# researchmm/MM-Diffusion

Hardware: AMD Instinct MI355X
Metric: denoising steps/sec (video+audio pair), 16x64x64 / 25600 (higher is better)
Workload: dtype bf16; 1 GPU; BASELINE configs[1]: Landscape base model (133.68M params), DDPM p_sample, timestep_respacing=250, per-GPU batch 4, 16x3x64x64 video + 1x25600 audio; global_batch=4, parallelism=batch-sharded x1, no in-loop collective, weights=key-seeded synthetic (mm_diffusion.synth), graph_replay=True, batch_lanes=2, finite=True, ranks_seen=1

## Files before the change

include/mmd.h:

```cpp
#ifndef MMD_H
#define MMD_H
#include <stdint.h>
#ifdef __cplusplus
extern "C" {
#endif

#define MMD_F32 0
#define MMD_BF16 1
#define MMD_OK 0
#define MMD_ERR_ARG (-1)
#define MMD_ERR_LAUNCH (-2)
#define MMD_ERR_UNSUPPORTED (-3)

int mmd_version(void);
const char* mmd_last_error(void);
int mmd_debug_install_crash_handler(void);

int mmd_graph_begin(void* stream);
int mmd_graph_end(void* stream, void** exec_out);
int mmd_graph_launch(void* exec, void* stream);
int mmd_graph_destroy(void* exec);
int mmd_stream_create(void** stream_out);
int mmd_stream_sync(void* stream);
int mmd_stream_destroy(void* stream);
int mmd_event_create(void** ev);
int mmd_event_record(void* ev, void* stream);
int mmd_stream_wait_event(void* stream, void* ev);
int mmd_event_elapsed_ms(void* ev_start, void* ev_stop, float* ms);
int mmd_event_destroy(void* ev);

int mmd_temb_fwd(const void* t, int t_kind, int N, int dim, const float* W0, const float* b0, const float* W2,
                 const float* b2, float* out_silu, float* out_raw, void* stream);

int mmd_linear_fwd(const float* x, const float* W, const float* b, float* y, int N, int K, int J, void* stream);

int64_t mmd_gn_workspace_bytes(int dtype, int C, int S, int Tn);
int mmd_gn_stats(int dtype, const void* x, int64_t ld, int C, int S, int Tn, int inner, int64_t outer_stride,
                 int64_t inner_stride, int64_t tstride, const float* gamma, const float* beta, const float* film,
                 int64_t film_ld, float eps, float* a_out, float* b_out, float* mr_out, void* workspace, void* stream);
int mmd_gn_finalize_stats(const float* rec, int64_t rec_ld, int C, int S, int Tn, const float* gamma, const float* beta,
                          const float* film, int64_t film_ld, float eps, float* a_out, float* b_out, float* mr_out, void* stream);
int mmd_gn_apply(int dtype, const void* x, int64_t ldx, void* y, int64_t ldy, int64_t rows, int C, int S, int Tn, int inner,
                 int64_t outer_stride, int64_t inner_stride, int64_t tstride, const float* a, const float* b, int act,
                 void* stream);
int mmd_add_rowbias(int dtype, void* x, int64_t ld, int64_t rows, int C, int64_t rows_per_sample, const float* e,
                    int64_t e_ld, void* stream);
int mmd_colsum_slices(int dtype, const void* dY, int64_t lddy, int S, int64_t Tn, int C, float* out, int64_t ldo, void* stream);

int mmd_conv_gemm(int dtype, const void* A, int64_t lda, const void* W, const float* bias, const void* R, int64_t ldr,
                  void* Y, int64_t ldy, int M, int Cout, int Cin, int ntaps, const int* taps, int D0, int D1, int D2, int tile,
                  void* stream);

int mmd_gn_conv1x1(int dtype, const void* A, int64_t lda, const float* gn_a, const float* gn_b, int act, int S,
                   int64_t rows_per_slice, const void* W, const float* bias, const void* R, int64_t ldr, void* Y, int64_t ldy,
                   int M, int Cout, int Cin, int tile, void* stream);

int mmd_gn_small(int dtype, const void* x, int64_t ldx, void* y, int64_t ldy, int C, int S, int Tn, int inner, int64_t outer_stride,
                 int64_t inner_stride, int64_t tstride, const float* gamma, const float* beta, float eps, int act, void* stream);

int mmd_gn_group(int dtype, const void* x, int64_t ldx, void* y, int64_t ldy, int C, int S, int Tn, int inner, int64_t outer_stride,
                 int64_t inner_stride, int64_t tstride, const float* gamma, const float* beta, const float* film, int64_t film_ld,
                 float eps, int act, float* a_out, float* b_out, float* mr_out, void* stream);

int mmd_zero(void* ptr, int64_t bytes, void* stream);

int mmd_conv_gemm_stats(int dtype, const void* A, int64_t lda, const void* W, const float* bias, const void* R, int64_t ldr,
                        void* Y, int64_t ldy, int M, int Cout, int Cin, int ntaps, const int* taps, int D0, int D1, int D2, int tile,
                        float* stats, int64_t stats_ld, void* stream);
int mmd_gn_conv1x1_stats(int dtype, const void* A, int64_t lda, const float* gn_a, const float* gn_b, int act, int S,
                         int64_t rows_per_slice, const void* W, const float* bias, const void* R, int64_t ldr, void* Y, int64_t ldy,
                         int M, int Cout, int Cin, int tile, float* stats, int64_t stats_ld, void* stream);

int mmd_gn_conv_gemm(int dtype, const void* A, int64_t lda, const float* gn_a, const float* gn_b, int act, int S,
                     int64_t rows_per_slice, const void* W, const float* bias, const void* R, int64_t ldr, void* Y, int64_t ldy,
                     int M, int Cout, int Cin, int ntaps, const int* taps, int D0, int D1, int D2, int tile, void* stream);

int64_t mmd_vconv2d1d_weight_bytes(int Cin);
int mmd_vconv2d1d_pack(const void* Ws, const void* Wt, void* out, int Cin, int Cout, void* stream);
int mmd_vconv2d1d(const void* X, int64_t ldx, const float* gn_a, const float* gn_b, int act, int S, int64_t rows_per_slice,
                  const void* Wf, const float* bias_s, const float* bias_t, void* Y, int64_t ldy, int N, int F, int H, int W,
                  int Cin, int Cout, float* stats, int64_t stats_ld, void* stream);

int64_t mmd_tattn_weight_bytes(int C, int with_pre);
int mmd_tattn_pack(const void* Wpre, const void* Wqkv, const void* Wproj, void* out, int C, void* stream);
int mmd_tattn_block(const void* X, int64_t ldx, const void* A, int64_t lda, void* MID, int64_t ldm, const void* Wf,
                    const float* bias_pre, const float* bias_qkv, const float* bias_proj, const float* gamma, const float* beta,
                    float eps, void* Y, int64_t ldy, int N, int F, int HW, int C, int heads, float* stats, int64_t stats_ld,
                    void* stream);

int64_t mmd_tconv_weight_bytes(int Cin, int Cout);
int mmd_tconv_pack(const void* W, void* out, int Cin, int Cout, void* stream);
int mmd_tconv(const void* X, int64_t ldx, const void* Wf, const float* bias, void* Y, int64_t ldy, int N, int F, int HW, int Cin,
              int Cout, float* stats, int64_t stats_ld, void* stream);

int mmd_aconv(const void* X, int64_t ldx, const void* W, const float* bias, const float* ga, const float* gb, int act, void* Y, int64_t ldy,
              int M, int L, int Cin, int Cout, int dil, float* stats, int64_t stats_ld, void* stream);

int mmd_attn_fwd(int dtype, const void* Q, int64_t ldq, int q_off, const void* KV, int64_t ldkv, int k_off, int v_off, void* O,
                 int64_t ldo, int heads, int ch, int nb, int G, int64_t q_rows_per_batch, int q_per_group,
                 int64_t k_rows_per_batch, int k_per_group, int win, const int* shift_dev, int impl, void* stream);
int mmd_attn_small_fwd(int dtype, const void* QKV, int64_t ld, void* O, int64_t ldo, int C, int heads, int S, int Tn, int inner,
                       int64_t outer_stride, int64_t inner_stride, int64_t tstride, void* stream);

int mmd_resample(int dtype, const void* x, int64_t ldx, void* y, int64_t ldy, int C, int NF, int H, int W, int fh, int fw,
                 int mode, float scale, void* stream);
int mmd_resample_stats(const void* x, int64_t ldx, void* y, int64_t ldy, int C, int NF, int H, int W, int fh, int fw, int mode,
                       float* stats, int64_t stats_ld, void* stream);
int mmd_copy2d(const void* x, int64_t ldx_bytes, void* y, int64_t ldy_bytes, int64_t rows, int64_t row_bytes, void* stream);

int mmd_stem_conv(int dtype, const float* x, const float* w, const float* bias, void* y, int64_t ldy, int N, int F, int Cin,
                  int H, int W, int Cout, int ntaps, const int* taps, void* stream);
int mmd_head_conv(int dtype, const void* x, int64_t ldx, const float* w, const float* bias, float* y, int N, int F, int Cin,
                  int H, int W, int Co, int ntaps, const int* taps, void* stream);
int64_t mmd_head_gemm_weight_bytes(int Cin);
int64_t mmd_head_gemm_workspace_bytes(int64_t M, int ntaps, int Co);
int mmd_head_gemm(const void* x, int64_t ldx, int64_t M, int Cin, const float* gn_a, const float* gn_b, int S, int64_t gn_rows, int act,
                  const void* wimg, float* P, int NO, void* stream);
int mmd_head_gather(const float* P, const float* bias, float* y, int N, int F, int H, int W, int Co, int ntaps, const int* taps,
                    void* stream);

int mmd_ddpm_update(const float* x, const float* model_out, const float* noise, float* out, float* x0_out, float* mean_out,
                    float* logvar_out, const float* tables, const int64_t* t, int T, int N, int F, int C, int HW, int flags,
                    void* stream);
int mmd_q_sample(const float* x0, const float* eps, float* out, const float* tab2, const int64_t* t, int T, int N,
                 int64_t per_sample, void* stream);

int64_t mmd_loss_workspace_bytes(int N);
int mmd_loss_terms(const float* x0, const float* xt, const float* model_out, const float* target, const float* tables,
                   const int64_t* t, int T, int N, int F, int C, int HW, int flags, float vb_scale, float* mse_out, float* vb_out,
                   void* workspace, void* stream);

int mmd_conv_wgrad(int dtype, const void* dY, int64_t lddy, const void* X, int64_t ldx, float* dW, float* db, int M, int Cout, int Cin,
                   int ntaps, const int* taps, int D0, int D1, int D2, int torch_layout, void* stream);
int mmd_pack_blocks(int Cout, int Cin, int nt);
int mmd_pack_conv_weights(int dtype, const void* descs_dev, int n, int total_blocks, void* stream);
int mmd_unpack_conv_grads(const void* descs_dev, int n, int total_blocks, void* stream);
int mmd_gn_bwd(int dtype, const void* x, int64_t ldx, const void* dy, int64_t lddy, void* dx, int64_t lddx, int64_t rows, int C, int S,
               int Tn, int inner, int64_t outer_stride, int64_t inner_stride, int64_t tstride, const float* a, const float* b,
               const float* mr, const float* gamma, const float* beta, const float* film, int64_t film_ld, int act, float* dgamma,
               float* dbeta, float* dfilm, int64_t dfilm_ld, float* workspace, void* stream);
int mmd_gn_bwd_ws0(int dtype, const void* x, int64_t ldx, const void* dy, int64_t lddy, void* dx, int64_t lddx, int64_t rows, int C, int S,
                   int Tn, int inner, int64_t outer_stride, int64_t inner_stride, int64_t tstride, const float* a, const float* b,
                   const float* mr, const float* gamma, const float* beta, const float* film, int64_t film_ld, int act, float* dgamma,
                   float* dbeta, float* dfilm, int64_t dfilm_ld, float* workspace, void* stream);
int mmd_attn_bwd(int dtype, const void* Q, int64_t ldq, int q_off, const void* KV, int64_t ldkv, int k_off, int v_off, const void* O,
                 int64_t ldo, const void* dO, int64_t lddo, void* dQ, int64_t lddq, int dq_off, void* dKV, int64_t lddkv, int dk_off,
                 int dv_off, float* lse_ws, float* dsum_ws, int heads, int ch, int nb, int G, int q_inner, int64_t q_outer,
                 int64_t q_istride, int64_t q_tstride, int q_total, int q_per_group, int k_inner, int64_t k_outer, int64_t k_istride,
                 int64_t k_tstride, int k_mod, int k_per_group, int win, const int* shift_dev, void* stream);
int mmd_attn_fwd_lse(int dtype, const void* Q, int64_t ldq, int q_off, const void* KV, int64_t ldkv, int k_off, int v_off, void* O,
                     int64_t ldo, int heads, int ch, int nb, int G, int64_t q_rows_per_batch, int q_per_group,
                     int64_t k_rows_per_batch, int k_per_group, int win, const int* shift_dev, float* lse2_out, void* stream);
int mmd_attn_bwd_mfma(const void* Q, int64_t ldq, int q_off, const void* KV, int64_t ldkv, int k_off, int v_off, const void* O,
                      int64_t ldo, const void* dO, int64_t lddo, void* dQ, int64_t lddq, int dq_off, void* dKV, int64_t lddkv,
// ... 35 lines not shown
```

mm-diffusion_amd/build.py:

```python
#!/usr/bin/env python3
import os
import subprocess
import sys

HERE = os.path.dirname(os.path.abspath(__file__))
SRC = os.path.join(HERE, "csrc")
OUT = os.path.join(HERE, "lib", "libmmd.so")
SOURCES = ["mmd_core.hip", "mmd_gemm.hip", "mmd_vconv.hip", "mmd_tattn.hip", "mmd_tconv.hip", "mmd_aconv.hip", "mmd_norm.hip", "mmd_attn.hip", "mmd_misc.hip", "mmd_bwd.hip", "mmd_attn_bwd.hip", "mmd_attn_bwd_mfma.hip"]
FLAGS = ["--offload-arch=gfx950", "-O3", "-std=c++17", "-fPIC", "-ffp-contract=fast", "-Wno-unused-result", "-Wno-inline-asm"]
FLAGS += os.environ.get("MMD_EXTRA_CXXFLAGS", "").split()
NO_PACKED_F32 = ["-Xclang", "-target-feature", "-Xclang", "-packed-fp32-ops"]
FLAGS += NO_PACKED_F32


def _stale():
    if not os.path.exists(OUT):
        return True
    t = os.path.getmtime(OUT)
    deps = [os.path.join(SRC, f) for f in os.listdir(SRC)] + [os.path.abspath(__file__)]
    return any(os.path.getmtime(d) > t for d in deps)


def _llvm_bin():
    cands = [os.environ.get("LLVM_BIN")]
    hipcc = os.environ.get("HIPCC", "/opt/rocm/bin/hipcc")
    try:
        out = subprocess.run([hipcc, "--print-prog-name=llvm-objdump"], stdout=subprocess.PIPE, stderr=subprocess.DEVNULL, timeout=60).stdout.decode().strip()
        if out and os.path.isabs(out):
            cands.append(os.path.dirname(out))
    except (OSError, subprocess.SubprocessError):
        pass
    cands += [os.path.join(os.path.dirname(os.path.dirname(os.path.realpath(hipcc))), "lib", "llvm", "bin"), "/opt/rocm/lib/llvm/bin"]
    for d in cands:
        if d and os.path.exists(os.path.join(d, "llvm-objdump")):
            return d
    raise RuntimeError("build check: llvm-objdump not found (looked in %s); set LLVM_BIN to the LLVM bin directory of the ROCm toolchain"
                       % ", ".join(str(d) for d in cands if d))


def _check_no_packed_f32(path):
    import re
    import tempfile
    llvm = _llvm_bin()
    with tempfile.TemporaryDirectory() as td:
        lib = os.path.join(td, "lib.so")
        os.symlink(os.path.abspath(path), lib)
        subprocess.check_call([os.path.join(llvm, "llvm-objdump"), "--offloading", lib], cwd=td, stdout=subprocess.DEVNULL, stderr=subprocess.DEVNULL)
        cos = sorted(f for f in os.listdir(td) if f.endswith("gfx950"))
        if len(cos) < len(SOURCES) - 1:
            raise RuntimeError("build check: expected >= %d gfx950 code objects in %s, found %d" % (len(SOURCES) - 1, path, len(cos)))
        asm = ""
        for f in cos:
            asm += subprocess.run([os.path.join(llvm, "llvm-objdump"), "-d", "--mcpu=gfx950", os.path.join(td, f)],
                                  stdout=subprocess.PIPE, stderr=subprocess.DEVNULL, check=True).stdout.decode(errors="replace")
    n_mfma = len(re.findall(r"\bv_mfma_", asm))
    bad = re.findall(r"\bv_pk_(?:add|mul|fma)_f32\b", asm)
    if n_mfma == 0:
        raise RuntimeError("build check: the disassembly of %s shows no v_mfma instruction - the check looked at the wrong object" % path)
    if bad:
        raise RuntimeError("build check: %d packed-fp32 instruction(s) (%s ...) in %s: the device pass ignored %s" %
                           (len(bad), bad[0], path, " ".join(NO_PACKED_F32)))


def _check_strip_asm(obj):
    import importlib.util
    spec = importlib.util.spec_from_file_location("strip_asm_check", os.path.join(os.path.dirname(HERE), "tools", "strip_asm_check.py"))
    chk = importlib.util.module_from_spec(spec)
    spec.loader.exec_module(chk)
    chk.LLVM = _llvm_bin()
    n, bad = chk.check(chk.disassemble(obj))
    if n == 0 or bad:
        raise RuntimeError("build check: conv1x1_strip_res_kernel: %d kernels checked, %d violations%s" % (n, len(bad), (": " + bad[0]) if bad else ""))


def build(force=False, verbose=True):
    if not force and not _stale():
        return OUT
    os.makedirs(os.path.dirname(OUT), exist_ok=True)
    hipcc = os.environ.get("HIPCC", "/opt/rocm/bin/hipcc")
    objs = []
    procs = []
    for s in SOURCES:
        o = os.path.join(HERE, "lib", s.replace(".hip", ".o"))
        objs.append(o)
        cmd = [hipcc, *FLAGS, "-c", os.path.join(SRC, s), "-o", o]
        procs.append((cmd, subprocess.Popen(cmd, stdout=subprocess.PIPE, stderr=subprocess.STDOUT)))
    for cmd, p in procs:
        out, _ = p.communicate()
        if p.returncode != 0:
            raise RuntimeError("hipcc failed: %s\n%s" % (" ".join(cmd), out.decode()))
        lines = out.decode().splitlines()
        text = "\n".join(ln for ln in lines if "'-packed-fp32-ops' is not a recognized feature" not in ln).strip()
        if verbose and text:
            print(text)
    tmp = OUT + ".tmp"
    cmd = [hipcc, "--offload-arch=gfx950", "-shared", "-fPIC", "-o", tmp, *objs]
    try:
        subprocess.check_call(cmd)
        _check_no_packed_f32(tmp)
        _check_strip_asm(os.path.join(HERE, "lib", "mmd_gemm.o"))
        os.replace(tmp, OUT)
    finally:
        if os.path.exists(tmp):
            os.remove(tmp)
    if verbose:
        print("built", OUT)
    return OUT


if __name__ == "__main__":
    build(force="--force" in sys.argv)
```

mm-diffusion_amd/csrc/mmd_common.h:

```cpp
#pragma once
#include <hip/hip_runtime.h>
#include <stdint.h>
#include <stdio.h>
#include <stdarg.h>
#include "../../include/mmd.h"

#define MMD_F32 0
#define MMD_BF16 1

#define MMD_OK 0
#define MMD_ERR_ARG (-1)
#define MMD_ERR_LAUNCH (-2)
#define MMD_ERR_UNSUPPORTED (-3)

typedef __attribute__((ext_vector_type(8))) __bf16 bf16x8;
typedef __attribute__((ext_vector_type(4))) __bf16 bf16x4;
typedef __attribute__((ext_vector_type(16))) float f32x16;
typedef __attribute__((ext_vector_type(4))) float f32x4;
typedef __attribute__((ext_vector_type(4))) uint32_t u32x4;
typedef __attribute__((ext_vector_type(2))) uint32_t u32x2;

int mmd_set_error(int code, const char* fmt, ...);
int mmd_check_launch(const char* what);

// ... 4 lines not shown

__device__ __forceinline__ float bf16_bits_to_f32(uint32_t bits16) { return __uint_as_float(bits16 << 16); }
__device__ __forceinline__ uint32_t f32_to_bf16_bits(float f) {
  uint32_t u = __float_as_uint(f);
  if ((u & 0x7fffffffu) > 0x7f800000u) return 0x7fc0u;
  u += 0x7fffu + ((u >> 16) & 1u);
  return u >> 16;
}
__device__ __forceinline__ uint32_t pack_bf16x2(float lo, float hi) {
  return f32_to_bf16_bits(lo) | (f32_to_bf16_bits(hi) << 16);
}

template <typename T> struct Elt;
template <> struct Elt<float> {
  static constexpr int EPV = 4;
  static constexpr int DT = MMD_F32;
  __device__ static __forceinline__ void unpack(const u32x4& v, float* f) {
#pragma unroll
    for (int i = 0; i < 4; ++i) f[i] = __uint_as_float(v[i]);
  }
  __device__ static __forceinline__ u32x4 pack(const float* f) {
    u32x4 v;
#pragma unroll
    for (int i = 0; i < 4; ++i) v[i] = __float_as_uint(f[i]);
    return v;
  }
  __device__ static __forceinline__ float ld(const void* p, int64_t i) { return ((const float*)p)[i]; }
  __device__ static __forceinline__ void st(void* p, int64_t i, float v) { ((float*)p)[i] = v; }
};
template <> struct Elt<__bf16> {
  static constexpr int EPV = 8;
  static constexpr int DT = MMD_BF16;
  __device__ static __forceinline__ void unpack(const u32x4& v, float* f) {
#pragma unroll
    for (int i = 0; i < 4; ++i) {
      f[2 * i] = __uint_as_float(v[i] << 16);
      f[2 * i + 1] = __uint_as_float(v[i] & 0xffff0000u);
    }
  }
  __device__ static __forceinline__ u32x4 pack(const float* f) {
    bf16x8 t;
#pragma unroll
    for (int i = 0; i < 8; ++i) t[i] = (__bf16)f[i];
    return __builtin_bit_cast(u32x4, t);
  }
  __device__ static __forceinline__ float ld(const void* p, int64_t i) {
    return bf16_bits_to_f32(((const uint16_t*)p)[i]);
  }
  __device__ static __forceinline__ void st(void* p, int64_t i, float v) {
    ((__bf16*)p)[i] = (__bf16)v;
  }
};

__device__ __forceinline__ float silu_f(float x) { return x * __builtin_amdgcn_rcpf(1.0f + __expf(-x)); }

__device__ __forceinline__ float wave_sum(float v) {
#pragma unroll
  for (int o = 32; o > 0; o >>= 1) v += __shfl_xor(v, o, 64);
  return v;
}
__device__ __forceinline__ double wave_sum_d(double v) {
#pragma unroll
  for (int o = 32; o > 0; o >>= 1) v += __shfl_xor(v, o, 64);
  return v;
}
__device__ __forceinline__ float wave_max(float v) {
#pragma unroll
  for (int o = 32; o > 0; o >>= 1) v = fmaxf(v, __shfl_xor(v, o, 64));
  return v;
}

template <int CTRL, int ROWS>
__device__ __forceinline__ float dpp_add(float v) {
  return v + __builtin_bit_cast(float, __builtin_amdgcn_update_dpp(0, __builtin_bit_cast(int, v), CTRL, ROWS, 0xf, false));
}
__device__ __forceinline__ float halfwave_total(float v) {
  v = dpp_add<0x128, 0xf>(v);
  v = dpp_add<0x124, 0xf>(v);
  v = dpp_add<0x122, 0xf>(v);
  v = dpp_add<0x121, 0xf>(v);
  return dpp_add<0x142, 0xa>(v);
}


static inline int cdiv(int64_t a, int64_t b) { return (int)((a + b - 1) / b); }

#define MMD_MAX_DEVICES 16
static inline int mmd_device_slot() {
  int d = 0;
  (void)hipGetDevice(&d);
  return d & (MMD_MAX_DEVICES - 1);
}
```

mm-diffusion_amd/csrc/mmd_gemm.hip:

```cpp
#include "mmd_common.h"

struct ConvGemmParams {
  const char* A; int64_t lda;
  const char* W;
  const float* bias;
  const char* R; int64_t ldr;
  char* Y; int64_t ldy;
  int M, Cout, Cin, ntaps;
  int D0, D1, D2;
  const float* gn_a; const float* gn_b;
  int gn_act, gn_S;
  int64_t gn_rows;
  float* stats; int64_t stats_ld;
  int taps[27 * 3];
};

template <int BM, int BN>
__device__ __forceinline__ void epilogue_stats(const ConvGemmParams& p, float (&sum)[BM / 64][8], float (&sq)[BM / 64][8], float* sP, int m0,
                                               int n0, int tid) {
  constexpr int CVN = BN / 8, NREC = BM / 64;
  const int lane = tid & 63, wave = tid >> 6, cg = tid % CVN;
#pragma unroll
  for (int r = 0; r < NREC; ++r)
#pragma unroll
// ... 1143 lines not shown
      __builtin_amdgcn_s_barrier();
      asm volatile("" ::: "memory");
      const int wslot = (c * NT + t) % NWS;
      if (t == NT - 1 && !more && p.R) {
#pragma unroll
        for (int ps = 0; ps < NPASS; ++ps)
          rres[ps] = *(const u32x4*)(e_co < p.Cout ? p.R + (row_of(e_rr + ps * RP) * p.ldr + e_co) * ES : (const char*)g_zero_page);
      }
      auto group = [&](int i) {
        const int t2 = (t + 2) % NT, c2 = c + (t + 2) / NT;
        if (i < 2) {
          if (c2 < nchunk) issue_w1((wslot + 2) % NWS, c2, t2, i);
          else dma_dummy();
        } else if (t < HJ) { if (more) issue_h((c + 1) & 1, c + 1, t); else dma_dummy(); }
        else if (t == NT - 1 && c + 2 < nchunk) issue_gn(c + 2);
        else dma_dummy();
      };
      constexpr int TOFF[9] = {-19, -18, -17, -1, 0, 1, 17, 18, 19};
      int toff = TOFF[t];
      asm volatile("" : "+s"(toff));
      const bool tr_on = GN && more && t >= 2 && t < 2 + NSLOT;
      compute(wslot, c & 1, toff, group, [&](int g) { if (tr_on) transform((c + 1) & 1, c + 1, t - 2, g, 1); });
    }
  }
  asm volatile("s_waitcnt vmcnt(0)" ::: "memory");
  __syncthreads();
  if (p.R) {
#pragma unroll
    for (int ps = 0; ps < NPASS; ++ps) LAUNDER4(rres[ps]);
  }

#pragma unroll
  for (int a = 0; a < 2; ++a)
#pragma unroll
    for (int b2 = 0; b2 < 2; ++b2) {
      const int ml = wr * 64 + b2 * 32 + l31;
#pragma unroll
      for (int q = 0; q < 4; ++q) {
        const int col = wc * 64 + a * 32 + 8 * q + 4 * half;
        f32x4 v = {acc[a][b2][4 * q], acc[a][b2][4 * q + 1], acc[a][b2][4 * q + 2], acc[a][b2][4 * q + 3]};
        *(f32x4*)(sC + ml * LDC + col) = v;
      }
    }
  __syncthreads();
  if (e_co < p.Cout) {
#pragma unroll
    for (int ps = 0; ps < NPASS; ++ps) {
      const int ml = e_rr + ps * RP;
      const int64_t m = row_of(ml);
      float v[8];
      const f32x4 c0 = *(const f32x4*)(sC + ml * LDC + e_cg * 8);
      const f32x4 c1 = *(const f32x4*)(sC + ml * LDC + e_cg * 8 + 4);
#pragma unroll
      for (int j = 0; j < 4; ++j) { v[j] = c0[j] + bs[j]; v[4 + j] = c1[j] + bs[4 + j]; }
      if (p.R) {
        float rf[EPV];
        Elt<T>::unpack(rres[ps], rf);
#pragma unroll
        for (int j = 0; j < EPV; ++j) v[j] += rf[j];
      }
      *(u32x4*)(p.Y + (m * p.ldy + e_co) * ES) = Elt<T>::pack(v);
    }
  }
}

#define STRIP_RES_LOAD(J2, off, base)                                                                                        \
  do {                                                                                                                       \
    if ((J2) == 0) asm volatile("global_load_dwordx4 v[248:251], %0, %1" :: "v"(off), "s"(base) : "v248", "v249", "v250", "v251");  \
    else asm volatile("global_load_dwordx4 v[252:255], %0, %1" :: "v"(off), "s"(base) : "v252", "v253", "v254", "v255");       \
  } while (0)
#define STRIP_RES_UNPACK_ASM(A, B, C, D)                                                                                     \
  "s_waitcnt vmcnt(%8)\n\tv_lshlrev_b32 %0, 16, " A "\n\tv_and_b32 %1, 0xffff0000, " A "\n\tv_lshlrev_b32 %2, 16, " B "\n\tv_and_b32 %3, 0xffff0000, " B \
  "\n\tv_lshlrev_b32 %4, 16, " C "\n\tv_and_b32 %5, 0xffff0000, " C "\n\tv_lshlrev_b32 %6, 16, " D "\n\tv_and_b32 %7, 0xffff0000, " D
#define STRIP_RES_WAIT(J2, rf, n)                                                                                            \
  do {                                                                                                                       \
    if ((J2) == 0)                                                                                                           \
      asm volatile(STRIP_RES_UNPACK_ASM("v248", "v249", "v250", "v251")                                                      \
                   : "=v"(rf[0]), "=v"(rf[1]), "=v"(rf[2]), "=v"(rf[3]), "=v"(rf[4]), "=v"(rf[5]), "=v"(rf[6]), "=v"(rf[7]) : "n"(n));  \
    else                                                                                                                     \
      asm volatile(STRIP_RES_UNPACK_ASM("v252", "v253", "v254", "v255")                                                      \
                   : "=v"(rf[0]), "=v"(rf[1]), "=v"(rf[2]), "=v"(rf[3]), "=v"(rf[4]), "=v"(rf[5]), "=v"(rf[6]), "=v"(rf[7]) : "n"(n));  \
  } while (0)
__host__ __device__ constexpr int wait_imm(int vm) { return (vm & 15) | ((vm >> 4) << 14) | 0x0070; }
template <int KS, int RF, int CC, int GNM, int STM, bool HR>
__device__ __forceinline__ void conv1x1_strip_body(const ConvGemmParams& p, const int nsplit) {
  constexpr int K = 64 * KS;
  constexpr int NCG = 4 * KS;
  constexpr int BR = 128 * RF;
  constexpr int NA = CC / 32;
  constexpr int GP = CC / 32;
  constexpr int PLANE_B = CC * 128, STAGE_B = KS * PLANE_B;
  constexpr bool PIPE = KS >= 4 && !(KS == 4 && HR);
  constexpr bool DEFER = KS > 2 || RF == 1;
  static_assert(RF == 2 || CC == 32, "one row fragment per wave: one sub-tile per chunk, deferred epilogue");
  extern __shared__ __attribute__((aligned(16))) char smem[];
  char* sW = smem;

  const int tid = threadIdx.x;
  const int lane = tid & 63;
  const int wave = __builtin_amdgcn_readfirstlane(tid >> 6);
  const int half = lane >> 5, l31 = lane & 31;

  const int nwg = gridDim.x;
  int wgid;
  {
    const int bid = blockIdx.x, q = nwg >> 3, r = nwg & 7, xcd = bid & 7;
    wgid = (xcd < r ? xcd * (q + 1) : r * (q + 1) + (xcd - r) * q) + (bid >> 3);
  }
  const int sp = wgid % nsplit, mt = wgid / nsplit;
  const int Cs = p.Cout / nsplit, cbase = sp * Cs, nchunk = Cs / CC;
  const int m0 = mt * BR;
  float* sBias = (float*)(smem + 2 * STAGE_B);
  float* sGN = sBias + ((Cs + 3) & ~3);
  float* sRec = sGN + (GNM != 0 ? 4 * K : 0);

  typedef const __attribute__((address_space(1))) void* gptr_t;
  typedef __attribute__((address_space(3))) void* lptr_t;
  const int lrow = lane >> 3, pc = lane & 7;
  const char* w_ptr[GP];
#pragma unroll
  for (int ih = 0; ih < GP; ++ih) {
    const int row = 8 * (ih * 4 + wave) + lrow;
    const int logical = pc ^ ((row >> 1) & 7);
    w_ptr[ih] = p.W + ((int64_t)(cbase + row) * K + logical * 8) * 2;
  }
  const unsigned lds0 = (unsigned)(uintptr_t)(lptr_t)sW;
  auto issue = [&](int stage, int ci) {
    const int64_t off = (int64_t)ci * CC * K * 2;
#pragma unroll
    for (int pl = 0; pl < KS; ++pl)
#pragma unroll
      for (int ih = 0; ih < GP; ++ih)
        asm volatile("s_mov_b32 m0, %1\n\ts_nop 0\n\tglobal_load_lds_dwordx4 %0, off"
                     :: "v"(w_ptr[ih] + off + pl * 128), "s"(lds0 + stage * STAGE_B + pl * PLANE_B + (ih * 4 + wave) * 1024) : "memory", "m0");
  };

  issue(0, 0);
  int rowc[RF];
  bool rok[RF];
  uint32_t yoff[RF], roff[RF];
  u32x4 xa[RF][NCG];
#pragma unroll
  for (int f = 0; f < RF; ++f) {
    const int row = m0 + wave * (32 * RF) + f * 32 + l31;
    rok[f] = row < p.M;
    rowc[f] = rok[f] ? row : p.M - 1;
    yoff[f] = (uint32_t)rowc[f] * (uint32_t)(p.ldy * 2) + 16 * half;
    roff[f] = (uint32_t)rowc[f] * (uint32_t)(p.ldr * 2) + 16 * half;
    if (p.ntaps == 1) {
      const char* ap = p.A + ((int64_t)rowc[f] * p.lda + half * 8) * 2;
#pragma unroll
      for (int cg = 0; cg < NCG; ++cg) xa[f][cg] = *(const u32x4*)(ap + cg * 32);
    } else {
      const int D12 = p.D1 * p.D2;
      const int q2 = rowc[f] % p.D2, q1 = (rowc[f] / p.D2) % p.D1, q0 = (rowc[f] / D12) % p.D0;
#pragma unroll
      for (int pl = 0; pl < KS; ++pl) {
        const int tap = (64 * pl) / p.Cin, ci0 = 64 * pl - tap * p.Cin;
        const int o0 = p.taps[3 * tap], o1 = p.taps[3 * tap + 1], o2 = p.taps[3 * tap + 2];
        const bool ok = (unsigned)(q0 + o0) < (unsigned)p.D0 && (unsigned)(q1 + o1) < (unsigned)p.D1 && (unsigned)(q2 + o2) < (unsigned)p.D2;
        const int64_t src = (int64_t)rowc[f] + (int64_t)o0 * D12 + o1 * p.D2 + o2;
        const char* ap = ok ? p.A + (src * p.lda + ci0 + half * 8) * 2 : (const char*)g_zero_row + half * 16;
#pragma unroll
        for (int c = 0; c < 4; ++c) xa[f][4 * pl + c] = *(const u32x4*)(ap + c * 32);
      }
    }
  }
  constexpr bool gn = GNM != 0;
// ... 96 lines not shown
    auto epi_step = [&](int s_, f32x16 (&ac)[RF], float (&kp)[2][2], int t, bool dma_between, bool last) __attribute__((always_inline)) {
      const int j2 = t / PJ, r = t % PJ;
      const int cb = s_ * 32;
      const int a = s_ % NA, par = (s_ / NA) & 1;
      if (r == 0) {
        if (j2 == 0) {
          eb[1][0] = *(const f32x4*)(sBias + cb + 16 + 8 * half);
          eb[1][1] = *(const f32x4*)(sBias + cb + 16 + 8 * half + 4);
        }
#pragma unroll
        for (int k = 0; k < 4; ++k) eu[k] = 0.f;
      }
      if (r < RF * SPU) {
        const int f = r / SPU, k = r % SPU;
        if (k < 4) {
          if (HR && k == 0) {
            if (last) STRIP_RES_WAIT(j2, erf, 2 * (NU - 1 - (j2 * RF + f)) + (j2 * RF + f));
            else if (dma_between) STRIP_RES_WAIT(j2, erf, 2 * (NU - 1) + D);
            else STRIP_RES_WAIT(j2, erf, 2 * (NU - 1));
          }
          const auto sw = __builtin_amdgcn_permlane32_swap(__float_as_uint(ac[f][8 * j2 + k]), __float_as_uint(ac[f][8 * j2 + 4 + k]), false, false);
          ev[k] = __uint_as_float(sw[0]) + eb[j2][0][k];
          ev[4 + k] = __uint_as_float(sw[1]) + eb[j2][1][k];
          if constexpr (HR) {
            ev[k] += erf[k];
            ev[4 + k] += erf[4 + k];
          }
        } else if (k == 4) {
          epk = Elt<__bf16>::pack(ev);
          *(u32x4*)(p.Y + (int64_t)(cbase + cb + 16 * j2) * 2 + yoff[f]) = epk;
          if (HR && !last) STRIP_RES_LOAD(j2, roff[f], p.R + (int64_t)(cbase + cb + 32 + 16 * j2) * 2);
        } else {
          const int q = k - 5;
          const float r0 = __uint_as_float(epk[q] << 16), r1 = __uint_as_float(epk[q] & 0xffff0000u);
          eu[q >> 1] += r0;
          eu[q >> 1] += r1;
          eu[2 + (q >> 1)] += r0 * r0;
          eu[2 + (q >> 1)] += r1 * r1;
        }
      } else {
        const int h = r - RF * SPU;
        if (h < 4) et[h] = halfwave_total(eu[h]);
        else {
          kp[j2][0] = (l31 & 1) ? et[1] : et[0];
          kp[j2][1] = (l31 & 1) ? et[3] : et[2];
          if (RF == 1) {
            float* d = sRec + ((l31 >> 1) == 8 ? (((par * 4 + wave) * (NA * 2) + a * 2 + j2) * 2 + half) * 4 + (l31 & 1) * 2 : 128 + lane * 2);
            d[0] = kp[j2][0];
            d[1] = kp[j2][1];
          }
        }
      }
    };
    auto block = [&](int s_, f32x16 (&an)[RF], f32x16 (&ap)[RF], float (&kp)[2][2], bool dma_between) __attribute__((always_inline)) {
#pragma unroll
      for (int ks = 0; ks < PF; ++ks) frag_read(s_, ks);
      epi_begin(s_ - 1);
      __builtin_amdgcn_sched_barrier(0);
#pragma unroll
      for (int i = 0; i < NM; ++i) {
        if (i % RF == 0 && i / RF + PF < NKS) frag_read(s_, i / RF + PF);
        mfma_one(i, an);
        __builtin_amdgcn_sched_barrier(0);
#pragma unroll
        for (int t = NSTEP * i / NM; t < NSTEP * (i + 1) / NM; ++t) epi_step(s_ - 1, ap, kp, t, dma_between, false);
        __builtin_amdgcn_sched_barrier(0);
      }
    };
    auto mfma_sub = [&](int s_, f32x16 (&ac)[RF]) __attribute__((always_inline)) {
#pragma unroll
      for (int ks = 0; ks < PF; ++ks) frag_read(s_, ks);
#pragma unroll
      for (int i = 0; i < NM; ++i) {
        if (i % RF == 0 && i / RF + PF < NKS) frag_read(s_, i / RF + PF);
        mfma_one(i, ac);
      }
    };
    auto epi = [&](int s_, f32x16 (&ac)[RF], float (&kp)[2][2], bool dma_between, bool last) __attribute__((always_inline)) {
      epi_begin(s_);
#pragma unroll
      for (int t = 0; t < NSTEP; ++t) epi_step(s_, ac, kp, t, dma_between, last);
    };
    auto commit = [&](int s_, float (&kp)[2][2]) __attribute__((always_inline)) {
      if (STM == 1 && wave_ok && (RF == 2 || (wave & 1) == 0) && (l31 >> 1) == 8) {
        const int a = s_ % NA, par = (s_ / NA) & 1;
#pragma unroll
        for (int j2 = 0; j2 < 2; ++j2) {
          const int col = cbase + s_ * 32 + 16 * j2 + 8 * half;
          float* d = p.stats + (rec * p.stats_ld + (col >> 2) + (l31 & 1)) * 2;
          float o0 = 0.f, o1 = 0.f;
          if (RF == 1) {
            const float* o = sRec + ((((par * 4 + wave + 1) * (NA * 2) + a * 2 + j2) * 2 + half) * 4 + (l31 & 1) * 2);
            o0 = o[0];
            o1 = o[1];
          }
          d[0] = kp[j2][0] + o0;
          d[1] = kp[j2][1] + o1;
        }
      }
    };
    auto boundary = [&](int c) __attribute__((always_inline)) {
      if (c == 1) __builtin_amdgcn_s_waitcnt(wait_imm((NA - 1) * NU * VM_U));
      else __builtin_amdgcn_s_waitcnt(wait_imm(NA * NU * VM_U));
      __builtin_amdgcn_s_barrier();
      asm volatile("" ::: "memory");
      issue((c + 1) & 1, c + 1 < nchunk ? c + 1 : nchunk - 1);
    };
    issue(1, nchunk > 1 ? 1 : 0);
    mfma_sub(0, acc[0]);
    for (int s1 = 1; s1 < NS; s1 += 2) {
      if (NA == 1) {
        boundary(s1);
        if (RF == 1 && s1 >= 2) commit(s1 - 2, keep[1]);
      }
      block(s1, acc[1], acc[0], keep[0], NA == 1);
      if (RF == 2) commit(s1 - 1, keep[0]);
      if (s1 + 1 < NS) {
        boundary((s1 + 1) / NA);
        if (RF == 1) commit(s1 - 1, keep[0]);
        block(s1 + 1, acc[0], acc[1], keep[1], true);
        if (RF == 2) commit(s1, keep[1]);
      }
    }
    auto tail = [&](f32x16 (&ac)[RF], float (&kp)[2][2], float (&kq)[2][2]) __attribute__((always_inline)) {
      epi(NS - 1, ac, kp, false, true);
      if (RF == 2) commit(NS - 1, kp);
      if (RF == 1 && STM == 1) {
        __builtin_amdgcn_s_waitcnt(wait_imm(63));
        __builtin_amdgcn_s_barrier();
        if (NS >= 2) commit(NS - 2, kq);
        commit(NS - 1, kp);
      }
    };
    if ((NS - 1) & 1) tail(acc[1], keep[1], keep[0]);
    else tail(acc[0], keep[0], keep[1]);
    asm volatile("s_waitcnt vmcnt(0)" ::: "memory");
  } else {
  for (int ci = 0; ci < nchunk; ++ci) {
    const int st = ci & 1;
    if (ci + 1 < nchunk) issue(st ^ 1, ci + 1);
    u32x4 outv[RF][2];
    float srec[2][2];
#pragma unroll
    for (int a = 0; a < NA; ++a) {
      const int cb = ci * CC + a * 32;
      u32x4 rres[RF][2];
      if constexpr (HR) {
#pragma unroll
        for (int f = 0; f < RF; ++f)
#pragma unroll
          for (int j2 = 0; j2 < 2; ++j2)
            rres[f][j2] = *(const u32x4*)(p.R + (int64_t)(cbase + cb + 16 * j2) * 2 + roff[f]);
        __builtin_amdgcn_sched_barrier(0);
      }
      f32x16 acc[RF];
#pragma unroll
      for (int f = 0; f < RF; ++f)
#pragma unroll
        for (int r = 0; r < 16; ++r) acc[f][r] = 0.f;
      const char* bW = sW + st * STAGE_B + (a * 32 + l31) * 128;
#pragma unroll
      for (int pl = 0; pl < KS; ++pl)
#pragma unroll
        for (int c = 0; c < 4; ++c) {
          const u32x4 fw = *(const u32x4*)(bW + pl * PLANE_B + (((2 * c + half) ^ xsw) * 16));
#pragma unroll
          for (int f = 0; f < RF; ++f) Mma<__bf16>::run(fw, xa[f][4 * pl + c], acc[f]);
        }
#pragma unroll
      for (int j2 = 0; j2 < 2; ++j2) {
        const int col = cbase + cb + 16 * j2 + 8 * half;
        const f32x4 b0 = *(const f32x4*)(sBias + cb + 16 * j2 + 8 * half), b1 = *(const f32x4*)(sBias + cb + 16 * j2 + 8 * half + 4);
        float u[16];
#pragma unroll
        for (int i = 0; i < 16; ++i) u[i] = 0.f;
#pragma unroll
        for (int f = 0; f < RF; ++f) {
          float v[8];
#pragma unroll
          for (int j = 0; j < 4; ++j) {
            const auto sw = __builtin_amdgcn_permlane32_swap(__float_as_uint(acc[f][8 * j2 + j]), __float_as_uint(acc[f][8 * j2 + 4 + j]),
                                                             false, false);
            v[j] = __uint_as_float(sw[0]);
            v[4 + j] = __uint_as_float(sw[1]);
          }
#pragma unroll
          for (int j = 0; j < 4; ++j) { v[j] += b0[j]; v[4 + j] += b1[j]; }
          if constexpr (HR) {
            float rf[8];
            Elt<__bf16>::unpack(rres[f][j2], rf);
#pragma unroll
            for (int j = 0; j < 8; ++j) v[j] += rf[j];
          }
          const u32x4 pk = Elt<__bf16>::pack(v);
          if (DEFER && a == NA - 1) outv[f][j2] = pk;
          else *(u32x4*)(p.Y + (int64_t)(cbase + cb + 16 * j2) * 2 + yoff[f]) = pk;
          if (STM != 0) {
            float rf[8];
            Elt<__bf16>::unpack(pk, rf);
#pragma unroll
            for (int j = 0; j < 4; ++j) {
              u[0] += rf[j];
              u[1] += rf[4 + j];
              u[2] += rf[j] * rf[j];
              u[3] += rf[4 + j] * rf[4 + j];
            }
          }
        }
        if (STM == 1) {
          const float t0 = halfwave_total(u[0]), t1 = halfwave_total(u[1]), t2 = halfwave_total(u[2]), t3 = halfwave_total(u[3]);
          const float msum = (l31 & 1) ? t1 : t0, msq = (l31 & 1) ? t3 : t2;
          if (RF == 1) {
            if ((l31 >> 1) == 8) {
              float* d = sRec + ((((ci & 1) * 4 + wave) * (NA * 2) + a * 2 + j2) * 2 + half) * 4 + (l31 & 1) * 2;
              d[0] = msum;
              d[1] = msq;
            }
            srec[j2][0] = msum;
            srec[j2][1] = msq;
          } else if (wave_ok && (l31 >> 1) == 8) {
            float* d = p.stats + (rec * p.stats_ld + (col >> 2) + (l31 & 1)) * 2;
            d[0] = msum;
            d[1] = msq;
          }
        }
      }
    }
    __builtin_amdgcn_s_waitcnt(0x0070);
    __builtin_amdgcn_s_barrier();
#pragma unroll
    for (int j2 = 0; DEFER && j2 < 2; ++j2) {
      const int col = cbase + ci * CC + (NA - 1) * 32 + 16 * j2 + 8 * half;
#pragma unroll
      for (int f = 0; f < RF; ++f)
        *(u32x4*)(p.Y + (int64_t)(cbase + ci * CC + (NA - 1) * 32 + 16 * j2) * 2 + yoff[f]) = outv[f][j2];
      if (RF == 1) {
        if (STM == 1 && wave_ok && (wave & 1) == 0 && (l31 >> 1) == 8) {
          const float* o = sRec + ((((ci & 1) * 4 + wave + 1) * (NA * 2) + (NA - 1) * 2 + j2) * 2 + half) * 4 + (l31 & 1) * 2;
          float* d = p.stats + (rec * p.stats_ld + (col >> 2) + (l31 & 1)) * 2;
          d[0] = srec[j2][0] + o[0];
          d[1] = srec[j2][1] + o[1];
        }
      }
    }
  }
  }
}

#define STRIP_LAUNCH_BOUNDS __launch_bounds__(256, (KS <= 2 ? (RF == 1 ? 4 : 3) : 2))
template <int KS, int RF, int CC, int GNM, int STM>
__global__ STRIP_LAUNCH_BOUNDS void conv1x1_strip_kernel(const ConvGemmParams p, const int nsplit) {
  conv1x1_strip_body<KS, RF, CC, GNM, STM, false>(p, nsplit);
}
template <int KS, int RF, int CC, int GNM, int STM>
__global__ STRIP_LAUNCH_BOUNDS __attribute__((amdgpu_num_vgpr(248))) void conv1x1_strip_res_kernel(const ConvGemmParams p, const int nsplit) {
  conv1x1_strip_body<KS, RF, CC, GNM, STM, true>(p, nsplit);
}

template <int KS, int RF, int CC, int GNM, int STM, bool HR>
static int launch_conv1x1_strip_res(const ConvGemmParams& p, hipStream_t st) {
  constexpr int BR = 128 * RF, STAGE_B = KS * CC * 128;
  const int rowblocks = cdiv(p.M, BR), nch = p.Cout / CC;
  static const int want_blocks = [] {
    const char* e = getenv("MMD_STRIP_BLOCKS");
    const int v = e ? atoi(e) : 0;
    return v > 0 ? v : 256;
  }();
  int nsplit = 1;
  for (int d = 1; d <= nch && d <= 16; ++d)
    if (nch % d == 0) {
      nsplit = d;
      if ((int64_t)rowblocks * d >= want_blocks) break;
    }
  const int Cs = p.Cout / nsplit;
  constexpr size_t REC_B = RF == 1 ? 2 * 4 * (CC / 32) * 2 * 32 * sizeof(float) : 0;
  const size_t lds = 2 * (size_t)STAGE_B + (size_t)((Cs + 3) & ~3) * 4 + (p.gn_a ? 4 * (size_t)(64 * KS) * 4 : 0) + REC_B;
  const size_t lds_max = 2 * (size_t)STAGE_B + 2048 * 4 + 4 * (size_t)(64 * KS) * 4 + REC_B;
  if (lds > lds_max) return mmd_set_error(MMD_ERR_UNSUPPORTED, "conv_gemm tile 131 (strip): %d output channels per block", Cs);
  static bool attr_done[MMD_MAX_DEVICES] = {};
  bool& attr_set = attr_done[mmd_device_slot()];
  if (!attr_set) {
    const void* kfn = HR ? (const void*)conv1x1_strip_res_kernel<KS, RF, CC, GNM, STM> : (const void*)conv1x1_strip_kernel<KS, RF, CC, GNM, STM>;
    hipError_t e = hipFuncSetAttribute(kfn, hipFuncAttributeMaxDynamicSharedMemorySize, (int)lds_max);
    if (e != hipSuccess) return mmd_set_error(MMD_ERR_LAUNCH, "conv1x1_strip: set LDS attr: %s", hipGetErrorString(e));
    attr_set = true;
  }
  if (HR) hipLaunchKernelGGL((conv1x1_strip_res_kernel<KS, RF, CC, GNM, STM>), dim3(rowblocks * nsplit), dim3(256), lds, st, p, nsplit);
  else hipLaunchKernelGGL((conv1x1_strip_kernel<KS, RF, CC, GNM, STM>), dim3(rowblocks * nsplit), dim3(256), lds, st, p, nsplit);
  return mmd_check_launch("conv1x1_strip");
}

template <int KS, int RF, int CC, int GNM, int STM>
static int launch_conv1x1_strip_mode(const ConvGemmParams& p, hipStream_t st) {
  return p.R ? launch_conv1x1_strip_res<KS, RF, CC, GNM, STM, true>(p, st) : launch_conv1x1_strip_res<KS, RF, CC, GNM, STM, false>(p, st);
}

template <int KS, int RF, int CC, int STM>
static int launch_conv1x1_strip_st(const ConvGemmParams& p, hipStream_t st) {
  if (!p.gn_a) return launch_conv1x1_strip_mode<KS, RF, CC, 0, STM>(p, st);
  return p.gn_act ? launch_conv1x1_strip_mode<KS, RF, CC, 2, STM>(p, st) : launch_conv1x1_strip_mode<KS, RF, CC, 1, STM>(p, st);
}

template <int KS, int RF, int CC>
static int launch_conv1x1_strip(const ConvGemmParams& p, hipStream_t st) {
  return p.stats ? launch_conv1x1_strip_st<KS, RF, CC, 1>(p, st) : launch_conv1x1_strip_st<KS, RF, CC, 0>(p, st);
}

static int dispatch_conv1x1_strip(const ConvGemmParams& p, hipStream_t st) {
  const int K = p.Cin * p.ntaps;
  const int rf = K <= 256 ? 2 : 1, cc = K <= 256 ? 64 : 32;
  if ((K != 128 && K != 256 && K != 384 && K != 512) || p.Cin % 64 != 0 || p.Cout % cc != 0 ||
      (int64_t)p.M * p.ldy * 2 >= 0xffffffffLL || (p.R && (int64_t)p.M * p.ldr * 2 >= 0xffffffffLL) || (p.gn_a && (p.ntaps != 1 || p.gn_rows < 128 * rf)) ||
      (p.ntaps == 1 && (p.taps[0] || p.taps[1] || p.taps[2])))
    return mmd_set_error(MMD_ERR_UNSUPPORTED, "conv_gemm tile 131 (strip): needs ntaps * Cin in {128, 256, 384, 512}, Cin %% 64 == 0, Cout %% %d == 0, "
                         "fused GroupNorm only for 1x1 convs with slices of >= %d rows (got Cin=%d ntaps=%d Cout=%d)", cc, 128 * rf, p.Cin, p.ntaps, p.Cout);
  if (K == 128) {
    static const bool rf1 = [] { const char* e = getenv("MMD_STRIP_K128_RF1"); return !(e && e[0] == '0'); }();
    if (rf1 && p.gn_a && p.gn_rows >= 16384 && p.ntaps == 1 && p.Cout % 32 == 0) return launch_conv1x1_strip<2, 1, 32>(p, st);
    return launch_conv1x1_strip<2, 2, 64>(p, st);
  }
  if (K == 256) return launch_conv1x1_strip<4, 2, 64>(p, st);
  if (K == 384) return launch_conv1x1_strip<6, 1, 32>(p, st);
  return launch_conv1x1_strip<8, 1, 32>(p, st);
}

template <typename T, bool GN>
static int launch_conv_gemm_halo(const ConvGemmParams& p, hipStream_t st) {
  bool taps_ok = p.ntaps <= 9;
  for (int t = 0; t < p.ntaps && taps_ok; ++t)
    taps_ok = p.taps[t * 3] == 0 && p.taps[t * 3 + 1] >= -1 && p.taps[t * 3 + 1] <= 1 && p.taps[t * 3 + 2] >= -1 && p.taps[t * 3 + 2] <= 1;
  if (!taps_ok || p.D1 % 8 != 0 || p.D2 % 16 != 0 || (int64_t)p.D0 * p.D1 * p.D2 != p.M || p.Cin % (8 * Elt<T>::EPV) != 0)
    return mmd_set_error(MMD_ERR_UNSUPPORTED, "conv_gemm tile 130 (halo): needs spatial taps (|dh|,|dw| <= 1), D1 %% 8 == 0, D2 %% 16 == 0, "
                         "full frames and Cin a multiple of one 128-byte K step");
  if (GN && (p.ntaps != 9 || p.gn_rows % ((int64_t)p.D1 * p.D2) != 0))
    return mmd_set_error(MMD_ERR_UNSUPPORTED, "conv_gemm tile 130 with fused GroupNorm: needs the nine spatial taps and slices of whole frames");
  const size_t lds = 2 * (size_t)(23 * 8 * 128) + 2 * (size_t)(128 * 128) + 336 + (GN ? 1024 : 0);
  static bool attr_done[MMD_MAX_DEVICES] = {};
  bool& attr_set = attr_done[mmd_device_slot()];
  if (!attr_set) {
    hipError_t e = hipFuncSetAttribute((const void*)conv_gemm_halo_kernel<T, GN>, hipFuncAttributeMaxDynamicSharedMemorySize, (int)lds);
    if (e != hipSuccess) return mmd_set_error(MMD_ERR_LAUNCH, "conv_gemm_halo: set LDS attr: %s", hipGetErrorString(e));
    attr_set = true;
  }
  const int grid = (p.M / 128) * cdiv(p.Cout, 128);
  hipLaunchKernelGGL((conv_gemm_halo_kernel<T, GN>), dim3(grid), dim3(256), lds, st, p);
  return mmd_check_launch("conv_gemm_halo");
}

template <bool GN>
static int launch_conv_gemm_halo16(const ConvGemmParams& p, hipStream_t st) {
  bool taps_ok = p.ntaps == 9;
  for (int t = 0; t < p.ntaps && taps_ok; ++t)
    taps_ok = p.taps[t * 3] == 0 && p.taps[t * 3 + 1] == t / 3 - 1 && p.taps[t * 3 + 2] == t % 3 - 1;
  if (!taps_ok || p.D1 % 16 != 0 || p.D2 % 16 != 0 || (int64_t)p.D0 * p.D1 * p.D2 != p.M || p.Cin % 64 != 0 ||
      ((int64_t)p.D1 * p.D2 - 1) * p.lda * 2 + (int64_t)p.Cin * 2 >= 0x7fffffffLL || (int64_t)128 * p.Cin * 9 * 2 >= 0x7fffffffLL)
    return mmd_set_error(MMD_ERR_UNSUPPORTED, "conv_gemm tile 133 (halo, 16 x 16 patches): needs the nine spatial taps in row-major (dh, dw) order, "
                         "D1 %% 16 == 0, D2 %% 16 == 0, full frames, Cin %% 64 == 0 and frames below 2 GB");
  if (GN && p.gn_rows % ((int64_t)p.D1 * p.D2) != 0)
    return mmd_set_error(MMD_ERR_UNSUPPORTED, "conv_gemm tile 133 with fused GroupNorm: needs slices of whole frames");
  constexpr size_t OPS_B = 2 * (size_t)(41 * 8 * 128) + 3 * (size_t)(128 * 128), C_B = 256 * 132 * sizeof(float);
  const size_t lds = (OPS_B > C_B ? OPS_B : C_B) + 1024 + 256;
  static bool attr_done[MMD_MAX_DEVICES] = {};
  bool& attr_set = attr_done[mmd_device_slot()];
  if (!attr_set) {
    hipError_t e = hipFuncSetAttribute((const void*)conv_gemm_halo16_kernel<GN>, hipFuncAttributeMaxDynamicSharedMemorySize, (int)lds);
    if (e != hipSuccess) return mmd_set_error(MMD_ERR_LAUNCH, "conv_gemm_halo16: set LDS attr: %s", hipGetErrorString(e));
    attr_set = true;
  }
  const int grid = (p.M / 256) * cdiv(p.Cout, 128);
  hipLaunchKernelGGL((conv_gemm_halo16_kernel<GN>), dim3(grid), dim3(512), lds, st, p);
  return mmd_check_launch("conv_gemm_halo16");
}

template <typename T>
static bool glds_desc_ok(const ConvGemmParams& p) {
  static const bool on = [] { const char* e = getenv("MMD_GEMM_DESC"); return !(e && e[0] == '0'); }();
  constexpr int ES = 16 / Elt<T>::EPV;
  int maxshift = 0;
  for (int t = 0; t < p.ntaps; ++t) {
    const int64_t sh = ((int64_t)p.taps[3 * t] * p.D1 * p.D2 + (int64_t)p.taps[3 * t + 1] * p.D2 + p.taps[3 * t + 2]) * p.lda * ES;
    if (sh > 0x3fffffff || sh < -0x3fffffff) return false;
    (void)maxshift;
  }
  return on && ((int64_t)p.M * p.lda + p.Cin) * ES < 0x7fffffffLL && (int64_t)128 * p.Cin * p.ntaps * ES < 0x7fffffffLL;
}

template <typename T>
static int launch_conv_gemm_glds(const ConvGemmParams& p, hipStream_t st) {
  const size_t lds = 128 * 132 * sizeof(float) + 336;
  static bool attr_done[MMD_MAX_DEVICES] = {};
  bool& attr_set = attr_done[mmd_device_slot()];
  if (!attr_set) {
    hipError_t e = hipFuncSetAttribute((const void*)conv_gemm_glds_kernel<T, false, 2, false>, hipFuncAttributeMaxDynamicSharedMemorySize, (int)lds);
    if (e == hipSuccess) e = hipFuncSetAttribute((const void*)conv_gemm_glds_kernel<T, true, 2, false>, hipFuncAttributeMaxDynamicSharedMemorySize, (int)lds);
    if (e == hipSuccess) e = hipFuncSetAttribute((const void*)conv_gemm_glds_kernel<T, true, 2, true>, hipFuncAttributeMaxDynamicSharedMemorySize, (int)lds);
    if (e != hipSuccess) return mmd_set_error(MMD_ERR_LAUNCH, "conv_gemm_glds: set LDS attr: %s", hipGetErrorString(e));
    attr_set = true;
  }
  const int grid = cdiv(p.M, 128) * cdiv(p.Cout, 128);
  if (p.Cin % (8 * Elt<T>::EPV) != 0) hipLaunchKernelGGL((conv_gemm_glds_kernel<T, false, 2, false>), dim3(grid), dim3(256), lds, st, p);
  else if (glds_desc_ok<T>(p)) hipLaunchKernelGGL((conv_gemm_glds_kernel<T, true, 2, true>), dim3(grid), dim3(256), lds, st, p);
  else hipLaunchKernelGGL((conv_gemm_glds_kernel<T, true, 2, false>), dim3(grid), dim3(256), lds, st, p);
  return mmd_check_launch("conv_gemm_glds");
}

template <typename T>
static int launch_conv_gemm_ring(const ConvGemmParams& p, hipStream_t st) {
  if (p.Cin % (8 * Elt<T>::EPV) != 0)
    return mmd_set_error(MMD_ERR_UNSUPPORTED, "conv_gemm tile 132 (deep ring): Cin must be a multiple of one 128-byte K step");
  const size_t lds = 8 * (size_t)(128 * 128) + 336;
  static bool attr_done[MMD_MAX_DEVICES] = {};
  bool& attr_set = attr_done[mmd_device_slot()];
  if (!attr_set) {
    hipError_t e = hipFuncSetAttribute((const void*)conv_gemm_glds_kernel<T, true, 4, false>, hipFuncAttributeMaxDynamicSharedMemorySize, (int)lds);
    if (e == hipSuccess) e = hipFuncSetAttribute((const void*)conv_gemm_glds_kernel<T, true, 4, true>, hipFuncAttributeMaxDynamicSharedMemorySize, (int)lds);
    if (e != hipSuccess) return mmd_set_error(MMD_ERR_LAUNCH, "conv_gemm_ring: set LDS attr: %s", hipGetErrorString(e));
    attr_set = true;
  }
  const int grid = cdiv(p.M, 128) * cdiv(p.Cout, 128);
  if (glds_desc_ok<T>(p)) hipLaunchKernelGGL((conv_gemm_glds_kernel<T, true, 4, true>), dim3(grid), dim3(256), lds, st, p);
  else hipLaunchKernelGGL((conv_gemm_glds_kernel<T, true, 4, false>), dim3(grid), dim3(256), lds, st, p);
  return mmd_check_launch("conv_gemm_ring");
}

template <typename T, int BM, int BN, bool GN>
static int launch_conv_gemm(const ConvGemmParams& p, hipStream_t st) {
  const size_t lds_ops = 2 * (size_t)(BM + BN) * ROWB;
  const size_t lds_c = (size_t)BM * (BN + 4) * sizeof(float);
  const size_t lds = (lds_ops > lds_c ? lds_ops : lds_c) + 336 + (GN ? 16 * 256 : 0);
  static bool attr_done[MMD_MAX_DEVICES] = {};
  bool& attr_set = attr_done[mmd_device_slot()];
  if (!attr_set) {
    hipError_t e = hipFuncSetAttribute((const void*)conv_gemm_kernel<T, BM, BN, GN>,
                                       hipFuncAttributeMaxDynamicSharedMemorySize, (int)lds);
    if (e != hipSuccess) return mmd_set_error(MMD_ERR_LAUNCH, "conv_gemm: set LDS attr: %s", hipGetErrorString(e));
    attr_set = true;
  }
  const int grid = cdiv(p.M, BM) * cdiv(p.Cout, BN);
  hipLaunchKernelGGL((conv_gemm_kernel<T, BM, BN, GN>), dim3(grid), dim3(256), lds, st, p);
  return mmd_check_launch("conv_gemm");
}

template <typename T>
static int dispatch_conv_gemm(const ConvGemmParams& p, int tile, hipStream_t st) {
  if (tile == 133) {
    if constexpr (Elt<T>::EPV == 8) return p.gn_a ? launch_conv_gemm_halo16<true>(p, st) : launch_conv_gemm_halo16<false>(p, st);
    else return mmd_set_error(MMD_ERR_UNSUPPORTED, "conv_gemm tile 133: bf16 only");
  }
  if (p.gn_a) {
    if (tile == 130) {
      if constexpr (Elt<T>::EPV == 8) return launch_conv_gemm_halo<T, true>(p, st);
      else return mmd_set_error(MMD_ERR_UNSUPPORTED, "conv_gemm tile 130 with fused GroupNorm: bf16 only");
    }
    if (tile == 128) return launch_conv_gemm<T, 128, 128, true>(p, st);
    return launch_conv_gemm<T, 64, 64, true>(p, st);
  }
  if (tile == 129) return launch_conv_gemm_glds<T>(p, st);
  if (tile == 132) return launch_conv_gemm_ring<T>(p, st);
  if (tile == 130) return launch_conv_gemm_halo<T, false>(p, st);
  if (tile == 128) return launch_conv_gemm<T, 128, 128, false>(p, st);
  return launch_conv_gemm<T, 64, 64, false>(p, st);
}

static int conv_gemm_impl(int dtype, const void* A, int64_t lda, const void* W, const float* bias, const void* R, int64_t ldr,
                          void* Y, int64_t ldy, int M, int Cout, int Cin, int ntaps, const int* taps, int D0, int D1, int D2,
                          int tile, const float* gn_a, const float* gn_b, int gn_act, int gn_S, int64_t gn_rows, float* stats,
                          int64_t stats_ld, void* stream) {
  const int epv = dtype == MMD_BF16 ? 8 : 4;
  MMD_REQUIRE(dtype == MMD_BF16 || dtype == MMD_F32, "conv_gemm: bad dtype %d", dtype);
  MMD_REQUIRE(A && W && Y && M > 0 && Cout > 0 && Cin > 0, "conv_gemm: null/empty argument");
  MMD_REQUIRE(ntaps >= 1 && ntaps <= 27 && taps, "conv_gemm: ntaps %d out of [1,27]", ntaps);
  MMD_REQUIRE(Cin % epv == 0, "conv_gemm: Cin %d must be a multiple of %d", Cin, epv);
  MMD_REQUIRE(Cout % 8 == 0, "conv_gemm: Cout %d must be a multiple of 8", Cout);
  MMD_REQUIRE(lda % epv == 0 && ldy % epv == 0 && (!R || ldr % epv == 0), "conv_gemm: row strides must be 16-byte multiples");
  MMD_REQUIRE(((uintptr_t)A | (uintptr_t)W | (uintptr_t)Y | (uintptr_t)R) % 16 == 0, "conv_gemm: pointers must be 16-byte aligned");
  MMD_REQUIRE(D0 > 0 && D1 > 0 && D2 > 0, "conv_gemm: bad position dims");
  MMD_REQUIRE(!gn_a || (gn_b && (ntaps == 1 || tile == 130 || tile == 133) && gn_S > 0 && gn_rows >= 128 && (Cin <= 256 || tile == 131 || tile == 130 || tile == 133) &&
                        (int64_t)gn_S * gn_rows == M),
              "gn_conv1x1 / gn_conv_gemm: needs contiguous slices of >= 128 rows covering M, Cin <= 256 unless tile 130 / 131, taps only with tile 130 "
              "(got S=%d rows=%ld Cin=%d M=%d ntaps=%d tile=%d)", gn_S, (long)gn_rows, Cin, M, ntaps, tile);
  ConvGemmParams p;
  p.A = (const char*)A; p.lda = lda; p.W = (const char*)W; p.bias = bias;
  p.R = (const char*)R; p.ldr = ldr; p.Y = (char*)Y; p.ldy = ldy;
  p.M = M; p.Cout = Cout; p.Cin = Cin; p.ntaps = ntaps; p.D0 = D0; p.D1 = D1; p.D2 = D2;
  p.gn_a = gn_a; p.gn_b = gn_b; p.gn_act = gn_act; p.gn_S = gn_S; p.gn_rows = gn_rows;
  MMD_REQUIRE(!stats || (M % 64 == 0 && Cout % 4 == 0 && stats_ld >= Cout / 4 && tile != 130 && tile != 133 && (uintptr_t)stats % 8 == 0),
              "conv_gemm: output statistics need M %% 64 == 0, Cout %% 4 == 0, stats_ld >= Cout / 4 (quads) and a row-tiled main loop (not tiles 130 / 133)");
  p.stats = stats; p.stats_ld = stats_ld;
  for (int i = 0; i < ntaps * 3; ++i) p.taps[i] = taps[i];
  hipStream_t st = (hipStream_t)stream;
  if (tile == 0) tile = (int64_t)cdiv(M, 128) * cdiv(Cout, 128) >= 320 ? 128 : 64;
  MMD_REQUIRE(tile == 64 || tile == 128 || ((tile == 129 || tile == 132) && !gn_a) || (tile == 130 && (!gn_a || dtype == MMD_BF16)) ||
                  ((tile == 131 || tile == 133) && dtype == MMD_BF16),
              "conv_gemm: tile must be 0, 64, 128, 129 (128 direct-to-LDS), 130 (halo-tile 3x3), 131 (row strip, bf16 1x1 convs) or 132 (129 with a "
              "four-slot ring for launches of few tiles)");
  if (tile == 131) return dispatch_conv1x1_strip(p, st);
  return dtype == MMD_BF16 ? dispatch_conv_gemm<__bf16>(p, tile, st) : dispatch_conv_gemm<float>(p, tile, st);
}

extern "C" int mmd_conv_gemm(int dtype, const void* A, int64_t lda, const void* W, const float* bias, const void* R, int64_t ldr,
                             void* Y, int64_t ldy, int M, int Cout, int Cin, int ntaps, const int* taps, int D0, int D1, int D2,
                             int tile, void* stream) {
  return conv_gemm_impl(dtype, A, lda, W, bias, R, ldr, Y, ldy, M, Cout, Cin, ntaps, taps, D0, D1, D2, tile, nullptr, nullptr, 0, 0,
                        0, nullptr, 0, stream);
}

extern "C" int mmd_conv_gemm_stats(int dtype, const void* A, int64_t lda, const void* W, const float* bias, const void* R, int64_t ldr,
                                   void* Y, int64_t ldy, int M, int Cout, int Cin, int ntaps, const int* taps, int D0, int D1, int D2,
                                   int tile, float* stats, int64_t stats_ld, void* stream) {
  MMD_REQUIRE(stats, "conv_gemm_stats: null statistics buffer");
  return conv_gemm_impl(dtype, A, lda, W, bias, R, ldr, Y, ldy, M, Cout, Cin, ntaps, taps, D0, D1, D2, tile, nullptr, nullptr, 0, 0,
                        0, stats, stats_ld, stream);
}

extern "C" int mmd_gn_conv1x1(int dtype, const void* A, int64_t lda, const float* gn_a, const float* gn_b, int act, int S,
                              int64_t rows_per_slice, const void* W, const float* bias, const void* R, int64_t ldr, void* Y,
                              int64_t ldy, int M, int Cout, int Cin, int tile, void* stream) {
  static const int tap0[3] = {0, 0, 0};
  MMD_REQUIRE(gn_a && gn_b, "gn_conv1x1: null GroupNorm affine");
  return conv_gemm_impl(dtype, A, lda, W, bias, R, ldr, Y, ldy, M, Cout, Cin, 1, tap0, 1, 1, 1, tile, gn_a, gn_b, act, S,
                        rows_per_slice, nullptr, 0, stream);
}

extern "C" int mmd_gn_conv1x1_stats(int dtype, const void* A, int64_t lda, const float* gn_a, const float* gn_b, int act, int S,
                                    int64_t rows_per_slice, const void* W, const float* bias, const void* R, int64_t ldr, void* Y,
                                    int64_t ldy, int M, int Cout, int Cin, int tile, float* stats, int64_t stats_ld, void* stream) {
  static const int tap0[3] = {0, 0, 0};
  MMD_REQUIRE(gn_a && gn_b && stats, "gn_conv1x1_stats: null GroupNorm affine / statistics buffer");
  return conv_gemm_impl(dtype, A, lda, W, bias, R, ldr, Y, ldy, M, Cout, Cin, 1, tap0, 1, 1, 1, tile, gn_a, gn_b, act, S,
                        rows_per_slice, stats, stats_ld, stream);
}

extern "C" int mmd_gn_conv_gemm(int dtype, const void* A, int64_t lda, const float* gn_a, const float* gn_b, int act, int S,
                                int64_t rows_per_slice, const void* W, const float* bias, const void* R, int64_t ldr, void* Y,
                                int64_t ldy, int M, int Cout, int Cin, int ntaps, const int* taps, int D0, int D1, int D2, int tile,
                                void* stream) {
  MMD_REQUIRE(gn_a && gn_b, "gn_conv_gemm: null GroupNorm affine");
  MMD_REQUIRE(tile == 130 || tile == 133, "gn_conv_gemm: the fused input GroupNorm of a conv with taps exists on the halo tiles (130 / 133) only");
  return conv_gemm_impl(dtype, A, lda, W, bias, R, ldr, Y, ldy, M, Cout, Cin, ntaps, taps, D0, D1, D2, tile, gn_a, gn_b, act, S,
                        rows_per_slice, nullptr, 0, stream);
}
```

mm-diffusion_amd/csrc/mmd_norm.hip:

```cpp
#include "mmd_common.h"

#define GN_GROUPS 32
typedef __attribute__((ext_vector_type(2))) double f64x2;

struct SliceGeom {
  int S, Tn, inner;
  int64_t outer_stride, inner_stride, tstride;
};

__device__ __forceinline__ int64_t slice_base(const SliceGeom& g, int s) {
  return (int64_t)(s / g.inner) * g.outer_stride + (int64_t)(s % g.inner) * g.inner_stride;
}
__device__ __forceinline__ int slice_of_row(const SliceGeom& g, int64_t m) {
  const int64_t o = m / g.outer_stride, rem = m % g.outer_stride;
  return (int)(o * g.inner + (rem / g.inner_stride) % g.inner);
}

template <typename T, bool ONE>
__global__ __launch_bounds__(256) void gn_partial_kernel(const char* __restrict__ x, int64_t ld, int C, SliceGeom g, int R,
                                                         double* __restrict__ part, int nchunks,
                                                         const float* __restrict__ gamma, const float* __restrict__ beta,
                                                         const float* __restrict__ film, int64_t film_ld, float eps,
                                                         float* __restrict__ a_out, float* __restrict__ b_out, float* __restrict__ mr_out) {
  constexpr int EPV = Elt<T>::EPV;
  constexpr int ES = 16 / EPV;
  __shared__ float s_sum[2048];
  __shared__ float s_sq[2048];
  __shared__ float s_mean[GN_GROUPS], s_rstd[GN_GROUPS];
  const int s = blockIdx.y, chunk = blockIdx.x, tid = threadIdx.x;
  const int CV = C / EPV;
  const int CVB = min(CV, 256);
  const int RPP = 256 / CVB;
  const int col0 = tid % CVB, rl = tid / CVB;
  const int j0 = chunk * R;
  const int j1 = min(j0 + R, g.Tn);
  const int64_t base = slice_base(g, s);
  const int cpg = C / GN_GROUPS;
  for (int cp = 0; cp < CV; cp += 256) {
  const int col = col0 + cp;
  if (col >= CV) break;
  float sum[EPV], sq[EPV];
#pragma unroll
  for (int j = 0; j < EPV; ++j) sum[j] = sq[j] = 0.f;
  float piv[EPV];
  {
    const int c0 = col * EPV;
    const int g0 = c0 / cpg;
    int gc = g0, rem = c0 - g0 * cpg;
#pragma unroll
    for (int e = 0; e < EPV; ++e) {
      piv[e] = Elt<T>::ld(x, base * ld + (int64_t)gc * cpg);
      if (++rem == cpg) { rem = 0; ++gc; }
    }
  }
  if (rl < RPP) {
    const char* xp = x + (base * ld + (int64_t)col * EPV) * ES;
    const int64_t rstride = g.tstride * ld * ES;
    for (int jb = j0 + rl; jb < j1; jb += 4 * RPP) {
      u32x4 v[4];
#pragma unroll
      for (int u = 0; u < 4; ++u) {
        const int j = jb + u * RPP;
        if (j < j1) v[u] = *(const u32x4*)(xp + (int64_t)j * rstride);
      }
#pragma unroll
      for (int u = 0; u < 4; ++u) {
        if (jb + u * RPP < j1) {
          float f[EPV];
          Elt<T>::unpack(v[u], f);
#pragma unroll
          for (int e = 0; e < EPV; ++e) { const float d = f[e] - piv[e]; sum[e] += d; sq[e] += d * d; }
        }
      }
    }
#pragma unroll
    for (int e = 0; e < EPV; ++e) {
      s_sum[rl * C + col * EPV + e] = sum[e];
      s_sq[rl * C + col * EPV + e] = sq[e];
    }
  }
  }
  __syncthreads();
  {
    const int gi = tid >> 3, k = tid & 7;
    const int n = RPP * cpg;
// ... 294 lines not shown
  int R = 4 * rpp;
  while (cdiv(Tn, R) > cap / 4 && R < 1024) R *= 2;
  return R;
}

extern "C" int64_t mmd_gn_workspace_bytes(int dtype, int C, int S, int Tn) {
  if (C <= 0 || S <= 0 || Tn <= 0) return 0;
  return (int64_t)S * cdiv(Tn, gn_rows_per_block(dtype, C, S, Tn)) * GN_GROUPS * 2 * sizeof(double);
}

extern "C" int mmd_gn_stats(int dtype, const void* x, int64_t ld, int C, int S, int Tn, int inner, int64_t outer_stride,
                            int64_t inner_stride, int64_t tstride, const float* gamma, const float* beta,
                            const float* film, int64_t film_ld, float eps, float* a_out, float* b_out, float* mr_out,
                            void* workspace, void* stream) {
  int rc = check_geom("gn_stats", dtype, C, S, Tn, inner);
  if (rc) return rc;
  MMD_REQUIRE(x && gamma && beta && a_out && b_out, "gn_stats: null pointer");
  MMD_REQUIRE(((uintptr_t)x) % 16 == 0 && ld % (dtype == MMD_BF16 ? 8 : 4) == 0, "gn_stats: x must be 16-byte aligned rows");
  SliceGeom g{S, Tn, inner, outer_stride, inner_stride, tstride};
  hipStream_t st = (hipStream_t)stream;
  const int R = gn_rows_per_block(dtype, C, S, Tn);
  const int nchunks = cdiv(Tn, R);
  if (nchunks == 1) {
    if (dtype == MMD_BF16)
      hipLaunchKernelGGL((gn_partial_kernel<__bf16, true>), dim3(1, S), dim3(256), 0, st, (const char*)x, ld, C, g, R, (double*)nullptr, 1,
                         gamma, beta, film, film_ld, eps, a_out, b_out, mr_out);
    else
      hipLaunchKernelGGL((gn_partial_kernel<float, true>), dim3(1, S), dim3(256), 0, st, (const char*)x, ld, C, g, R, (double*)nullptr, 1,
                         gamma, beta, film, film_ld, eps, a_out, b_out, mr_out);
    return mmd_check_launch("gn_stats_one");
  }
  MMD_REQUIRE(workspace && ((uintptr_t)workspace) % 16 == 0, "gn_stats: 16-byte aligned workspace required for multi-block slices");
  dim3 grid(nchunks, S);
  if (dtype == MMD_BF16)
    hipLaunchKernelGGL((gn_partial_kernel<__bf16, false>), grid, dim3(256), 0, st, (const char*)x, ld, C, g, R, (double*)workspace, nchunks,
                       gamma, beta, film, film_ld, eps, a_out, b_out, (float*)nullptr);
  else
    hipLaunchKernelGGL((gn_partial_kernel<float, false>), grid, dim3(256), 0, st, (const char*)x, ld, C, g, R, (double*)workspace, nchunks,
                       gamma, beta, film, film_ld, eps, a_out, b_out, (float*)nullptr);
  rc = mmd_check_launch("gn_partial");
  if (rc) return rc;
  hipLaunchKernelGGL(gn_finalize_kernel, dim3(S), dim3(1024), 0, st, (const char*)x, dtype, ld, g, (const double*)workspace, nchunks, C, Tn, gamma, beta,
                     film, film_ld, eps, a_out, b_out, mr_out);
  return mmd_check_launch("gn_finalize");
}

__global__ __launch_bounds__(256) void gn_finalize_rec_kernel(const float* __restrict__ rec, int64_t rec_ld, int C, int S, int Tn,
                                                              const float* __restrict__ gamma, const float* __restrict__ beta,
                                                              const float* __restrict__ film, int64_t film_ld, float eps,
                                                              float* __restrict__ a_out, float* __restrict__ b_out, float* __restrict__ mr_out) {
  __shared__ double s_a[4], s_b[4];
  const int gi = blockIdx.x, s = blockIdx.y, tid = threadIdx.x;
  const int cpg = C / GN_GROUPS, qpg = cpg / 4;
  const int nrec = Tn / 64;
  const float* base = rec + ((int64_t)s * nrec * rec_ld + (int64_t)gi * qpg) * 2;
  const int total = nrec * qpg;
  const int c = gi * cpg + min(tid, cpg - 1);
  const float gv = gamma[c], bv0 = beta[c];
  float fsc = 0.f, fsh = 0.f;
  if (film) {
    fsc = film[(int64_t)s * film_ld + c];
    fsh = film[(int64_t)s * film_ld + C + c];
  }
  double a[4] = {0.0, 0.0, 0.0, 0.0}, b[4] = {0.0, 0.0, 0.0, 0.0};
  for (int i = tid; i < total; i += 1024) {
#pragma unroll
    for (int u = 0; u < 4; ++u) {
      const int k = i + 256 * u;
      const int kk = min(k, total - 1);
      const int r = kk / qpg, cq = kk - r * qpg;
      const float2 v = *(const float2*)(base + ((int64_t)r * rec_ld + cq) * 2);
      const double m = k < total ? 1.0 : 0.0;
      a[u] += m * (double)v.x;
      b[u] += m * (double)v.y;
    }
  }
  double ta = (a[0] + a[1]) + (a[2] + a[3]), tb = (b[0] + b[1]) + (b[2] + b[3]);
  ta = wave_sum_d(ta);
  tb = wave_sum_d(tb);
  if ((tid & 63) == 0) { s_a[tid >> 6] = ta; s_b[tid >> 6] = tb; }
  __syncthreads();
  if (tid < cpg) {
    const double sa = (s_a[0] + s_a[1]) + (s_a[2] + s_a[3]), sb = (s_b[0] + s_b[1]) + (s_b[2] + s_b[3]);
    const double cnt = (double)Tn * (double)cpg;
    const double mean = sa / cnt;
    double var = sb / cnt - mean * mean;
    if (var < 0.0) var = 0.0;
    const float mean_f = (float)mean, rstd_f = (float)(1.0 / sqrt(var + (double)eps));
    if (mr_out && tid == 0) {
      mr_out[((int64_t)s * GN_GROUPS + gi) * 2] = mean_f;
      mr_out[((int64_t)s * GN_GROUPS + gi) * 2 + 1] = rstd_f;
    }
    float av = rstd_f * gv;
    float bv = bv0 - mean_f * av;
    if (film) {
      const float sc = 1.f + fsc;
      av *= sc;
      bv = bv * sc + fsh;
    }
    a_out[(int64_t)s * C + c] = av;
    b_out[(int64_t)s * C + c] = bv;
  }
}

extern "C" int mmd_gn_finalize_stats(const float* rec, int64_t rec_ld, int C, int S, int Tn, const float* gamma, const float* beta,
                                     const float* film, int64_t film_ld, float eps, float* a_out, float* b_out, float* mr_out,
                                     void* stream) {
  MMD_REQUIRE(rec && gamma && beta && a_out && b_out, "gn_finalize_stats: null pointer");
  MMD_REQUIRE(C > 0 && C % (4 * GN_GROUPS) == 0 && C / GN_GROUPS <= 256 && rec_ld >= C / 4,
              "gn_finalize_stats: channel count %d (groups of whole quads: a multiple of 128; ld %ld quads)", C, (long)rec_ld);
  MMD_REQUIRE(S > 0 && Tn > 0 && Tn % 64 == 0, "gn_finalize_stats: slices must be multiples of 64 rows (S=%d Tn=%d)", S, Tn);
  hipLaunchKernelGGL(gn_finalize_rec_kernel, dim3(GN_GROUPS, S), dim3(256), 0, (hipStream_t)stream, rec, rec_ld, C, S, Tn, gamma, beta,
                     film, film_ld, eps, a_out, b_out, mr_out);
  return mmd_check_launch("gn_finalize_stats");
}

template <typename T>
__global__ __launch_bounds__(256) void gn_group_kernel(const char* __restrict__ x, int64_t ldx, char* __restrict__ y, int64_t ldy, int C,
                                                       SliceGeom g, const float* __restrict__ gamma, const float* __restrict__ beta,
                                                       const float* __restrict__ film, int64_t film_ld, float eps, int act,
                                                       float* __restrict__ a_out, float* __restrict__ b_out, float* __restrict__ mr_out) {
  constexpr int ES = sizeof(T), MAXI = 16;
  __shared__ float s_red[2][4];
  __shared__ float s_ab[2][64];
  const int gi = blockIdx.x, s = blockIdx.y, tid = threadIdx.x;
  const int cpg = C / GN_GROUPS, qpg = cpg / 4, items = g.Tn * qpg;
  const int64_t base = slice_base(g, s);
  const char* xg = x + (int64_t)gi * cpg * ES;
  float f[MAXI][4];
#pragma unroll
  for (int j = 0; j < MAXI; ++j) {
    const int i = tid + 256 * j;
    if (i < items) {
      const int r = i / qpg, k = i - r * qpg;
      const char* q = xg + ((base + (int64_t)r * g.tstride) * ldx + 4 * k) * ES;
      if constexpr (ES == 2) {
        const u32x2 v = *(const u32x2*)q;
        f[j][0] = __uint_as_float(v[0] << 16); f[j][1] = __uint_as_float(v[0] & 0xffff0000u);
        f[j][2] = __uint_as_float(v[1] << 16); f[j][3] = __uint_as_float(v[1] & 0xffff0000u);
      } else {
        const f32x4 v = *(const f32x4*)q;
        f[j][0] = v[0]; f[j][1] = v[1]; f[j][2] = v[2]; f[j][3] = v[3];
      }
    } else {
      f[j][0] = f[j][1] = f[j][2] = f[j][3] = 0.f;
    }
  }
  auto block_sum = [&](float v, int slot) {
    v = wave_sum(v);
    if ((tid & 63) == 0) s_red[slot][tid >> 6] = v;
    __syncthreads();
    return (s_red[slot][0] + s_red[slot][1]) + (s_red[slot][2] + s_red[slot][3]);
  };
  float t = 0.f;
#pragma unroll
  for (int j = 0; j < MAXI; ++j) t += (f[j][0] + f[j][1]) + (f[j][2] + f[j][3]);
  const float inv_cnt = 1.f / ((float)g.Tn * (float)cpg);
  const float mean = block_sum(t, 0) * inv_cnt;
  t = 0.f;
#pragma unroll
  for (int j = 0; j < MAXI; ++j)
    if (tid + 256 * j < items) {
      const float d0 = f[j][0] - mean, d1 = f[j][1] - mean, d2 = f[j][2] - mean, d3 = f[j][3] - mean;
      t += (d0 * d0 + d1 * d1) + (d2 * d2 + d3 * d3);
    }
  const float var = block_sum(t, 1) * inv_cnt;
  const float rstd = (float)(1.0 / sqrt((double)var + (double)eps));
  if (tid < cpg) {
    const int c = gi * cpg + tid;
    float av = rstd * gamma[c];
    float bv = beta[c] - mean * av;
    if (film) {
      const float sc = 1.f + film[(int64_t)s * film_ld + c];
      av *= sc;
      bv = bv * sc + film[(int64_t)s * film_ld + C + c];
    }
    if (a_out) {
      a_out[(int64_t)s * C + c] = av;
      b_out[(int64_t)s * C + c] = bv;
    }
    s_ab[0][tid] = av;
// ... 110 lines not shown
```

mm-diffusion_amd/mm_diffusion/_hip.py:

```python
import ctypes as C
import gc
import os

import torch

_HERE = os.path.dirname(os.path.abspath(__file__))
LIB_PATH = os.environ.get("MMD_LIB") or os.path.join(os.path.dirname(_HERE), "lib", "libmmd.so")

F32, BF16 = 0, 1
_lib = None

i32, i64, f32, vp = C.c_int, C.c_int64, C.c_float, C.c_void_p


_PROTOS = {
    "mmd_version": (C.c_int, []),
    "mmd_last_error": (C.c_char_p, []),
    "mmd_debug_install_crash_handler": (i32, []),
    "mmd_graph_begin": (i32, [vp]),
    "mmd_graph_end": (i32, [vp, C.POINTER(vp)]),
    "mmd_graph_launch": (i32, [vp, vp]),
    "mmd_graph_destroy": (i32, [vp]),
    "mmd_stream_create": (i32, [C.POINTER(vp)]),
    "mmd_stream_sync": (i32, [vp]),
    "mmd_stream_destroy": (i32, [vp]),
    "mmd_event_create": (i32, [C.POINTER(vp)]),
    "mmd_event_record": (i32, [vp, vp]),
    "mmd_stream_wait_event": (i32, [vp, vp]),
    "mmd_event_elapsed_ms": (i32, [vp, vp, C.POINTER(f32)]),
    "mmd_event_destroy": (i32, [vp]),
    "mmd_temb_fwd": (i32, [vp, i32, i32, i32, vp, vp, vp, vp, vp, vp, vp]),
    "mmd_linear_fwd": (i32, [vp, vp, vp, vp, i32, i32, i32, vp]),
    "mmd_gn_workspace_bytes": (i64, [i32, i32, i32, i32]),
    "mmd_gn_stats": (i32, [i32, vp, i64, i32, i32, i32, i32, i64, i64, i64, vp, vp, vp, i64, f32, vp, vp, vp, vp, vp]),
    "mmd_gn_small": (i32, [i32, vp, i64, vp, i64, i32, i32, i32, i32, i64, i64, i64, vp, vp, f32, i32, vp]),
    "mmd_gn_group": (i32, [i32, vp, i64, vp, i64, i32, i32, i32, i32, i64, i64, i64, vp, vp, vp, i64, f32, i32, vp, vp, vp, vp]),
    "mmd_gn_apply": (i32, [i32, vp, i64, vp, i64, i64, i32, i32, i32, i32, i64, i64, i64, vp, vp, i32, vp]),
    "mmd_add_rowbias": (i32, [i32, vp, i64, i64, i32, i64, vp, i64, vp]),
    "mmd_colsum_slices": (i32, [i32, vp, i64, i32, i64, i32, vp, i64, vp]),
    "mmd_conv_gemm": (i32, [i32, vp, i64, vp, vp, vp, i64, vp, i64, i32, i32, i32, i32, C.POINTER(i32), i32, i32, i32, i32, vp]),
    "mmd_gn_conv1x1": (i32, [i32, vp, i64, vp, vp, i32, i32, i64, vp, vp, vp, i64, vp, i64, i32, i32, i32, i32, vp]),
    "mmd_conv_gemm_stats": (i32, [i32, vp, i64, vp, vp, vp, i64, vp, i64, i32, i32, i32, i32, C.POINTER(i32), i32, i32, i32, i32, vp, i64, vp]),
    "mmd_gn_conv1x1_stats": (i32, [i32, vp, i64, vp, vp, i32, i32, i64, vp, vp, vp, i64, vp, i64, i32, i32, i32, i32, vp, i64, vp]),
    "mmd_gn_conv_gemm": (i32, [i32, vp, i64, vp, vp, i32, i32, i64, vp, vp, vp, i64, vp, i64, i32, i32, i32, i32, C.POINTER(i32), i32, i32, i32, i32, vp]),
    "mmd_tconv_weight_bytes": (i64, [i32, i32]),
    "mmd_tconv_pack": (i32, [vp, vp, i32, i32, vp]),
    "mmd_tconv": (i32, [vp, i64, vp, vp, vp, i64, i32, i32, i32, i32, i32, vp, i64, vp]),
    "mmd_aconv": (i32, [vp, i64, vp, vp, vp, vp, i32, vp, i64, i32, i32, i32, i32, i32, vp, i64, vp]),
    "mmd_tattn_weight_bytes": (i64, [i32, i32]),
    "mmd_tattn_pack": (i32, [vp, vp, vp, vp, i32, vp]),
    "mmd_tattn_block": (i32, [vp, i64, vp, i64, vp, i64, vp, vp, vp, vp, vp, vp, f32, vp, i64, i32, i32, i32, i32, i32, vp, i64, vp]),
    "mmd_vconv2d1d_weight_bytes": (i64, [i32]),
    "mmd_vconv2d1d_pack": (i32, [vp, vp, vp, i32, i32, vp]),
    "mmd_vconv2d1d": (i32, [vp, i64, vp, vp, i32, i32, i64, vp, vp, vp, vp, i64, i32, i32, i32, i32, i32, i32, vp, i64, vp]),
    "mmd_zero": (i32, [vp, i64, vp]),
    "mmd_gn_finalize_stats": (i32, [vp, i64, i32, i32, i32, vp, vp, vp, i64, f32, vp, vp, vp, vp]),
    "mmd_attn_fwd": (i32, [i32, vp, i64, i32, vp, i64, i32, i32, vp, i64, i32, i32, i32, i32, i64, i32, i64, i32, i32, vp, i32, vp]),
    "mmd_attn_small_fwd": (i32, [i32, vp, i64, vp, i64, i32, i32, i32, i32, i32, i64, i64, i64, vp]),
    "mmd_resample": (i32, [i32, vp, i64, vp, i64, i32, i32, i32, i32, i32, i32, i32, f32, vp]),
    "mmd_resample_stats": (i32, [vp, i64, vp, i64, i32, i32, i32, i32, i32, i32, i32, vp, i64, vp]),
    "mmd_copy2d": (i32, [vp, i64, vp, i64, i64, i64, vp]),
    "mmd_stem_conv": (i32, [i32, vp, vp, vp, vp, i64, i32, i32, i32, i32, i32, i32, i32, C.POINTER(i32), vp]),
    "mmd_head_conv": (i32, [i32, vp, i64, vp, vp, vp, i32, i32, i32, i32, i32, i32, i32, C.POINTER(i32), vp]),
    "mmd_head_gemm_weight_bytes": (i64, [i32]),
    "mmd_head_gemm_workspace_bytes": (i64, [i64, i32, i32]),
    "mmd_head_gemm": (i32, [vp, i64, i64, i32, vp, vp, i32, i64, i32, vp, vp, i32, vp]),
    "mmd_head_gather": (i32, [vp, vp, vp, i32, i32, i32, i32, i32, i32, C.POINTER(i32), vp]),
    "mmd_ddpm_update": (i32, [vp, vp, vp, vp, vp, vp, vp, vp, vp, i32, i32, i32, i32, i32, i32, vp]),
    "mmd_loss_workspace_bytes": (i64, [i32]),
    "mmd_loss_terms": (i32, [vp, vp, vp, vp, vp, vp, i32, i32, i32, i32, i32, i32, f32, vp, vp, vp, vp]),
    "mmd_conv_wgrad": (i32, [i32, vp, i64, vp, i64, vp, vp, i32, i32, i32, i32, C.POINTER(i32), i32, i32, i32, i32, vp]),
    "mmd_gn_bwd": (i32, [i32, vp, i64, vp, i64, vp, i64, i64, i32, i32, i32, i32, i64, i64, i64, vp, vp, vp, vp, vp, vp, i64, i32, vp, vp, vp, i64, vp, vp]),
    "mmd_gn_bwd_ws0": (i32, [i32, vp, i64, vp, i64, vp, i64, i64, i32, i32, i32, i32, i64, i64, i64, vp, vp, vp, vp, vp, vp, i64, i32, vp, vp, vp, i64, vp, vp]),
    "mmd_attn_bwd": (i32, [i32, vp, i64, i32, vp, i64, i32, i32, vp, i64, vp, i64, vp, i64, i32, vp, i64, i32, i32, vp, vp, i32, i32, i32, i32,
                           i32, i64, i64, i64, i32, i32, i32, i64, i64, i64, i32, i32, i32, vp, vp]),
    "mmd_timestep_embedding": (i32, [vp, i32, i32, i32, vp, vp]),
    "mmd_attn_fwd_lse": (i32, [i32, vp, i64, i32, vp, i64, i32, i32, vp, i64, i32, i32, i32, i32, i64, i32, i64, i32, i32, vp, vp, vp]),
    "mmd_attn_bwd_mfma": (i32, [vp, i64, i32, vp, i64, i32, i32, vp, i64, vp, i64, vp, i64, i32, vp, i64, i32, i32, vp, vp, i32, i32, i32, i32,
                                i64, i32, i64, i32, i32, vp, vp]),
    "mmd_attn_small_bwd": (i32, [i32, vp, i64, vp, i64, vp, i64, i32, i32, i32, i32, i32, i64, i64, i64, vp]),
    "mmd_ddim_update": (i32, [vp, vp, vp, vp, vp, vp, vp, vp, i32, i32, i32, i32, i32, i32, f32, vp]),
    "mmd_lincomb_t": (i32, [vp, vp, vp, vp, vp, vp, vp, i32, i64, vp]),
    "mmd_lincomb": (i32, [vp, f32, vp, f32, vp, f32, vp, i64, vp]),
    "mmd_cast": (i32, [vp, i32, vp, i32, f32, i64, vp]),
    "mmd_ddpm_update_bwd": (i32, [vp, vp, vp, vp, vp, vp, vp, i32, i32, i64, i32, vp]),
    "mmd_abs_quantile": (i32, [vp, i32, i64, f32, vp, vp]),
    "mmd_clamp_scale": (i32, [vp, vp, f32, i32, i64, vp]),
    "mmd_dpm_err": (i32, [vp, vp, vp, f32, f32, i32, i64, vp, vp]),
    "mmd_bilinear_concat": (i32, [vp, vp, vp, i32, i32, i32, i32, i32, i32, vp]),
    "mmd_bilinear_concat_rows": (i32, [i32, vp, vp, vp, i32, i32, i32, i32, i32, i32, i32, vp]),
    "mmd_pack_conv_weights": (i32, [i32, vp, i32, i32, vp]),
    "mmd_pack_blocks": (i32, [i32, i32, i32]),
    "mmd_unpack_conv_grads": (i32, [vp, i32, i32, vp]),
    "mmd_loss_terms_bwd": (i32, [vp, vp, vp, vp, vp, vp, i32, i32, i32, i32, i32, i32, f32, vp, vp, vp, vp]),
    "mmd_silu": (i32, [i32, vp, vp, vp, i64, vp]),
    "mmd_dropout": (i32, [i32, vp, vp, f32, vp, i64, vp]),
    "mmd_mse_grad": (i32, [vp, vp, vp, vp, i32, i64, vp]),
    "mmd_adamw_step": (i32, [vp, vp, vp, vp, vp, i64, f32, f32, f32, f32, f32, i32, f32, vp]),
    "mmd_q_sample": (i32, [vp, vp, vp, vp, vp, i32, i32, i64, vp]),
}
EXPORTS = tuple(_PROTOS)


class MMDError(RuntimeError):
    pass


def lib():
    global _lib
    if _lib is None:
        if not os.path.exists(LIB_PATH):
            raise MMDError(f"{LIB_PATH} not found - build it with `python mm-diffusion_amd/build.py` "
                           "(the MI355X HIP path has no CPU/torch fallback)")
        l = C.CDLL(LIB_PATH)
        for name, (res, args) in _PROTOS.items():
            fn = getattr(l, name)
            fn.restype, fn.argtypes = res, args
        _lib = l
    return _lib


def call(name, *args):
    rc = getattr(lib(), name)(*args)
    if rc != 0:
        raise MMDError(f"{name} failed ({rc}): {lib().mmd_last_error().decode()}")

# ... 153 lines not shown
```

mm-diffusion_amd/mm_diffusion/engine.py:

```python
import os

import torch

from . import _hip as H
from . import ops
from .ops import Geom


_EMB_ON_AUDIO_STREAM = os.environ.get("MMD_EMB_AUX", "1") != "0"
_POOL_NOREUSE = os.environ.get("MMD_POOL_NOREUSE") == "1"
_UP_LOWRES = os.environ.get("MMD_UP_LOWRES", "1") != "0"
_CROSS_SERIAL = os.environ.get("MMD_CROSS_SERIAL", "1") != "0"
_RESAMPLE_STATS = os.environ.get("MMD_RESAMPLE_STATS", "1") != "0"


class _Pool:

    def __init__(self, device):
        self.device = device
        self.free = []
        self.all = []

    def get(self, nbytes):
        nbytes = (int(nbytes) + 255) // 256 * 256
        best = None
        for i, raw in enumerate(self.free):
            sz = raw.numel()
            if sz >= nbytes and sz <= 2 * nbytes + 65536 and (best is None or sz < self.free[best].numel()):
                best = i
        if best is not None:
            return self.free.pop(best)
        raw = torch.empty(nbytes, dtype=torch.uint8, device=self.device)
        self.all.append(raw)
        return raw

    def put(self, raw):
        if not _POOL_NOREUSE:
            self.free.append(raw)

    def total_bytes(self):
        return sum(r.numel() for r in self.all)


class UNetEngine:
    def __init__(self, model, N, dtype, device):
        if not torch.cuda.is_available():
            raise H.MMDError("no HIP device visible: the MI355X path cannot run (no CPU fallback)")
        H.lib()
        self.model, self.N, self.dtype, self.device = model, N, dtype, torch.device(device)
        self.F, self.Cv_in, self.H0, self.W0 = model.video_size
        self.Ca_in, self.L0 = model.audio_size
        self.mc = model.model_channels
        self.params = {k: v for k, v in model.named_parameters()}
        for k, v in self.params.items():
            if v.device.type != "cuda":
                raise H.MMDError(f"parameter {k} is on {v.device}: move the model to the GPU first (model.to('cuda'))")
        self._sig = self._signature()
        self.pools = [_Pool(self.device), _Pool(self.device)]
        mode = os.environ.get("MMD_GN_EPILOGUE", "1")
        self.rec_enabled = mode == "2" or (mode != "0" and dtype == torch.bfloat16)
        self._recs = {}
        self._gn_small = os.environ.get("MMD_GN_SMALL", "1") != "0"
        self._vconv_fused = self._tattn_fused = self._tconv = self._aconv = dtype == torch.bfloat16
        self._deferred = []
        H.reap()
        self._aux, self._side = H.Stream(self.device), H.Stream(self.device)
        self.aux = self._aux.torch
        self.side = self._side.torch
        self.keep = []
        self.plan = []
        self.graph = None
        self._build()

    def _signature(self):
        return tuple((p.data_ptr(), p._version) for p in self.params.values())

    def stale(self):
        return self._sig != self._signature()

    def _alloc(self, rows, C, dtype=None, stats=False, unit=64):
        dtype = dtype or self.dtype
        es = torch.empty(0, dtype=dtype).element_size()
        pool = self.pools[ops.cur_sid]
        raw = pool.get(rows * C * es)
        t = raw[: rows * C * es].view(dtype).view(rows, C)
        t._raw, t._pool = raw, pool
        if stats and self.rec_enabled and rows % 64 == 0 and unit % 64 == 0 and C % 4 == 0:
            rec = self._alloc(rows // 64, C // 2, torch.float32)
            self._recs[raw.untyped_storage().data_ptr()] = dict(rec=rec, view=rec.view(rows // 64, C // 4, 2), ptr=t.data_ptr(), es=es,
                                                                rows=rows, C=C, cover=[])
        return t

    def _release(self, *ts):
        for t in ts:
            if t is not None and hasattr(t, "_raw"):
                ent = self._recs.pop(t._raw.untyped_storage().data_ptr(), None)
                if ent is not None:
                    self._release(ent["rec"])
                t._pool.put(t._raw)
                del t._raw

    def _rec_slice(self, t):
        ent = self._recs.get(t.untyped_storage().data_ptr())
        if ent is None or t.stride(0) != ent["C"] or t.shape[0] != ent["rows"]:
            return None, 0
        c0 = (t.data_ptr() - ent["ptr"]) // ent["es"]
        return (ent, c0) if 0 <= c0 and c0 + t.shape[1] <= ent["C"] else (None, 0)

    def _stats_for(self, out, perm_unit=0):
        ent, c0 = self._rec_slice(out)
        if ent is None or c0 % 4 or out.shape[1] % 4:
            return None
        ent["perm_unit"] = max(ent.get("perm_unit", 0), perm_unit)
        ent["cover"].append((c0, c0 + out.shape[1]))
        return ent["view"][:, c0 // 4:(c0 + out.shape[1]) // 4, :]

    def _has_stats(self, out):
        return self._rec_slice(out)[0] is not None

    def _resample_stats(self, out):
        if not _RESAMPLE_STATS or self.dtype != torch.bfloat16:
            return None
        ent, c0 = self._rec_slice(out)
        if ent is None or c0 % 8 or out.shape[1] % 8 or ent["C"] % 8:
            return None
        return self._stats_for(out)

    def _stats_kw(self, out):
        rec = self._stats_for(out)
        return {} if rec is None else {"stats": rec}

    def _rec_ready(self, x, geom):
        ent, c0 = self._rec_slice(x)
        if (ent is None or geom.inner != 1 or geom.tstride != 1 or geom.outer_stride != geom.Tn or geom.Tn % 64 or geom.S * geom.Tn != x.shape[0]
                or c0 % 4 or x.shape[1] % 128):
            return None
        if ent.get("perm_unit", 0) and geom.Tn % ent["perm_unit"]:
            return None
        need, pos = c0 + x.shape[1], c0
        for lo, hi in sorted(ent["cover"]):
            if lo > pos:
                break
            pos = max(pos, hi)
        return ent["view"][:, c0 // 4:need // 4, :] if pos >= need else None

    def _static(self, shape, dtype):
        t = torch.zeros(shape, dtype=dtype, device=self.device)
        self.keep.append(t)
        return t

    def _packed(self, kind, key, make):
        cache = self.model.__dict__.setdefault("_wcache", {})
        if cache.get("sig") != self._sig:
            cache.clear()
            cache["sig"] = self._sig
        k = (kind, key, self.dtype if kind == "gemm" else None, str(self.device))
        t = cache.get(k)
        if t is None:
            t = cache[k] = make()
        self.keep.append(t)
        return t

    def _f32(self, key):
        return self._packed("f32", key, lambda: self.params[key].detach().float().contiguous())

    def _gemm_w(self, key):
        return self._packed("gemm", key, lambda: ops.pack_conv_weight(self.params[key].detach().float(), self.dtype))

    def _edge_w(self, key):
        return self._packed("edge", key, lambda: ops.pack_edge_weight(self.params[key].detach()))

    def _temporal(self, Hh):
        if ops.HALO_CANDIDATE:
            return dict(taps=ops.TAPS_TEMPORAL_D1, dims=(self.N, self.F, Hh * Hh))
        return dict(taps=ops.TAPS_TEMPORAL, dims=(self.F, Hh * Hh, 1))

    def _gn(self, x, prefix, geom, act, film=None, out=None):
        C = x.shape[1]
        if film is None and self._gn_small and ops.gn_small_ok(x, geom):
            y = self._alloc(x.shape[0], C) if out is None else out
            return ops.gn_small(x, self._f32(prefix + ".GroupNorm.weight"), self._f32(prefix + ".GroupNorm.bias"), geom, act=act, out=y)
        if ops.gn_group_ok(x, geom) and self._rec_ready(x, geom) is None:
            y = self._alloc(x.shape[0], C) if out is None else out
            return ops.gn_group(x, self._f32(prefix + ".GroupNorm.weight"), self._f32(prefix + ".GroupNorm.bias"), geom, film=film, out=y, act=act)
        a, b = self._gn_affine(x, prefix, geom, film)
        y = self._alloc(x.shape[0], C) if out is None else out
        ops.gn_apply(x, a, b, geom, act=act, out=y)
        self._release(a, b)
        return y

    def _gn_affine(self, x, prefix, geom, film):
        C = x.shape[1]
        a = self._alloc(geom.S, C, torch.float32)
        b = self._alloc(geom.S, C, torch.float32)
        gamma, beta = self._f32(prefix + ".GroupNorm.weight"), self._f32(prefix + ".GroupNorm.bias")
        rec = self._rec_ready(x, geom)
        if rec is not None:
            ops.gn_finalize_stats(rec, gamma, beta, geom, film=film, a=a, b=b)
        elif ops.gn_group_ok(x, geom):
            ops.gn_group(x, gamma, beta, geom, film=film, a=a, b=b)
        else:
            ws = self._alloc(ops.gn_workspace_bytes(x, geom) // 8, 1, torch.float64)
            ops.gn_stats(x, gamma, beta, geom, film=film, a=a, b=b, ws=ws)
            self._release(ws)
        return a, b

    def _gn_pw(self, x, gn_prefix, geom, act, wkey, bkey, film=None, residual=None, out=None):
        C = x.shape[1]
        Cout = self.params[wkey].shape[0]
        will_emit = True if (out is not None and self._has_stats(out)) else None
        if not ops.gn_fusable(geom, C, Cout, x, will_emit, act):
            n1 = self._gn(x, gn_prefix, geom, act, film=film)
            y = self._pw(n1, wkey, bkey, residual=residual, out=out)
            self._release(n1)
            return y
        a, b = self._gn_affine(x, gn_prefix, geom, film)
        y = self._alloc(x.shape[0], Cout) if out is None else out
        ops.gn_conv1x1(x, a, b, geom, act, self._gemm_w(wkey), self._f32(bkey), residual=residual, out=y, **self._stats_kw(y))
        self._release(a, b)
        return y

    def _pw(self, x, wkey, bkey, residual=None, out=None):
        y = self._alloc(x.shape[0], self.params[wkey].shape[0]) if out is None else out
        return ops.conv_gemm(x, self._gemm_w(wkey), self._f32(bkey), residual=residual, out=y, **self._stats_kw(y))

    def _self_attn(self, x, prefix, kind, Hh, out, pre=None, no_proj=False):
        N, F, C = self.N, self.F, x.shape[1]
        heads = self.model.num_heads
        ch = C // heads
        rows = x.shape[0]
        if kind == "spatial":
            geom = Geom.spatial(N, F, Hh * Hh)
        elif kind == "temporal":
            geom = Geom.temporal(N, F, Hh * Hh)
        else:
            geom = Geom.per_sample(N, rows // N)
        if kind == "temporal" and self._tattn_fused and ops.tattn_fused_ok(x, heads, N, F, Hh * Hh):
            pk = None
            if pre is not None:
                att, sp = pre
                mid = self._alloc(rows, C)
                pk = (att, self._f32(sp + ".proj_out.bias"), mid)
            wf = self._packed("tattn_pre" if pre is not None else "tattn", prefix, lambda: ops.tattn_pack(
                self._gemm_w(prefix + ".qkv.weight"), self._gemm_w(prefix + ".proj_out.weight"),
                wpre=self._gemm_w(pre[1] + ".proj_out.weight") if pre is not None else None))
            ops.tattn_block(x, wf, self._f32(prefix + ".qkv.bias"), self._f32(prefix + ".proj_out.bias"),
                            self._f32(prefix + ".norm.GroupNorm.weight"), self._f32(prefix + ".norm.GroupNorm.bias"), heads, N, F, Hh * Hh,
                            out=out, stats=self._stats_for(out, perm_unit=rows // N), pre=pk)
            if pk is not None:
                self._release(pk[2])
            return out
        qkv = self._gn_pw(x, prefix + ".norm", geom, False, prefix + ".qkv.weight", prefix + ".qkv.bias")
        att = self._alloc(rows, C)
        if kind == "temporal":
            if F > 32:
                raise H.MMDError(f"temporal attention over {F} frames: the short-sequence kernel handles <= 32")
            ops.attn_small(qkv, att, C, heads, geom)
        else:
            T = geom.Tn
            G = F if kind == "spatial" else 1
            ops.attn(qkv, qkv, att, heads, ch, N, G, G * T, T, G * T, T, 1)
        self._release(qkv)
        if no_proj:
            return att
        self._pw(att, prefix + ".proj_out.weight", prefix + ".proj_out.bias", residual=x, out=out)
        self._release(att)
        return out

    def _res(self, v, a, layer, Hh, L, out_v=None, out_a=None):
        N, F = self.N, self.F
        p, cin, cout = layer["prefix"], layer["cin"], layer["cout"]
        ss = self.model.use_scale_shift_norm
        film = self.emb_all[:, layer["emb_off"]: layer["emb_off"] + (2 * cout if ss else cout)]
        fh = 2 if (layer["up"] or layer["down"]) else 1
        Ho = Hh // 2 if layer["down"] else (Hh * 2 if layer["up"] else Hh)
        Lo = L // 4 if layer["down"] else (L * 4 if layer["up"] else L)
        mode = 0 if layer["down"] else 1

        def stream(x, mod, rows_in, rows_out, out):
            vid = mod == "video"
# ... 133 lines not shown
        self._release(*self._deferred)
        self._deferred = []
        sh = self.shift_dev[layer["shift_idx"]: layer["shift_idx"] + 1] if layer["shift"] else None
        ops.cur_sid = 0
        vatt = self._alloc(N * F * HW, C)
        ops.attn(vqkv, aqkv, vatt, heads, ch, N, F, F * HW, HW, L, apf, win, shift_dev=sh)
        if _CROSS_SERIAL:
            ops.record_sync(0, 1)
            ops.cur_sid = 1
            aatt = self._alloc(N * L, C)
            ops.attn(aqkv, vqkv, aatt, heads, ch, N, F, L, apf, F * HW, HW, win, shift_dev=sh)
            self._release(aqkv)
            self._deferred.append(vqkv)
        else:
            ops.cur_sid = 1
            aatt = self._alloc(N * L, C)
            ops.attn(aqkv, vqkv, aatt, heads, ch, N, F, L, apf, F * HW, HW, win, shift_dev=sh)
            ops.record_sync(0, 1)
            ops.record_sync(1, 0)
            self._release(vqkv, aqkv)
        ops.cur_sid = 0
        vo = out_v if out_v is not None else self._alloc(N * F * HW, C, stats=True, unit=F * HW)
        self._pw(vatt, p + ".video_proj_out.video_conv.weight", p + ".video_proj_out.video_conv.bias", residual=v, out=vo)
        self._release(vatt)
        ops.cur_sid = 1
        ao = out_a if out_a is not None else self._alloc(N * L, C, stats=True, unit=L)
        self._pw(aatt, p + ".audio_proj_out.audio_conv.weight", p + ".audio_proj_out.audio_conv.bias", residual=a, out=ao)
        self._release(aatt)
        ops.cur_sid, ops.cur_tag = 0, ""
        return vo, ao

    def _build(self):
        m, N, F, dt = self.model, self.N, self.F, self.dtype
        self._deferred = []
        arch_in, arch_mid, arch_out = m._arch
        if self.H0 != self.W0:
            raise H.MMDError("square frames only (the reference's avg-pool/upsample path is exercised on H == W)")
        self.x_video = self._static((N, F, self.Cv_in, self.H0, self.W0), torch.float32)
        self.x_audio = self._static((N, self.Ca_in, self.L0), torch.float32)
        self.t_i64 = self._static((N,), torch.int64)
        self.t_f32 = self._static((N,), torch.float32)
        self.out_video = self._static((N, F, m.video_out_channels, self.H0, self.W0), torch.float32)
        self.out_audio = self._static((N, m.audio_out_channels, self.L0), torch.float32)
        nshift, off = 0, 0
        Ws, bs = [], []
        for blk in arch_in + [arch_mid] + arch_out:
            for layer in blk:
                if layer["kind"] == "cross" and layer["shift"]:
                    layer["shift_idx"] = nshift
                    nshift += 1
                if layer["kind"] == "res":
                    layer["emb_off"] = off
                    W = self.params[layer["prefix"] + ".emb_layers.1.weight"]
                    Ws.append(W.detach().float())
                    bs.append(self.params[layer["prefix"] + ".emb_layers.1.bias"].detach().float())
                    off += W.shape[0]
        self.nshift = nshift
        self.shift_dev = self._static((max(nshift, 1),), torch.int32)
        self._shift_up = H.Staged(self.shift_dev)
        self.emb_W = torch.cat(Ws).contiguous()
        self.emb_b = torch.cat(bs).contiguous()
        self.emb_silu = self._static((N, self.mc), torch.float32)
        self.emb_all = self._static((N, off), torch.float32)

        def record(t_tensor):
            plan = []
            with ops.recording(plan):
                self._record(t_tensor, arch_in, arch_mid, arch_out)
            return plan

        self.plan = record(self.t_i64)
        self.plan_f32 = [(fn, (self.t_f32.data_ptr(), 2) + args[2:], name, meta, sid, tag) if name == "mmd_temb_fwd"
                         else (fn, args, name, meta, sid, tag) for fn, args, name, meta, sid, tag in self.plan]

    def _record(self, t_tensor, arch_in, arch_mid, arch_out):
        m, N, F, dt = self.model, self.N, self.F, self.dtype
        mc = self.mc
        ops.cur_sid = 0
        ops.record_sync(0, 1)
        ops.cur_sid = 1 if _EMB_ON_AUDIO_STREAM else 0
        ops.temb(t_tensor, mc, self._f32("time_embed.0.weight"), self._f32("time_embed.0.bias"),
                 self._f32("time_embed.2.weight"), self._f32("time_embed.2.bias"), self.emb_silu)
        ops.linear(self.emb_silu, self.emb_W, self.emb_b, self.emb_all)
        ops.cur_sid = 0
        film_joined = not _EMB_ON_AUDIO_STREAM
        if not _EMB_ON_AUDIO_STREAM:
            ops.record_sync(0, 1)

        skip_cols = []
        ch = arch_mid[-1]["cout"]
        for layers in arch_out:
            ich = layers[0]["skip_ch"]
            skip_cols.append((ch, ich))
            ch = layers[-1]["cout"] if layers[-1]["kind"] == "res" else layers[-1]["ch"]

        Hh, L = self.H0, self.L0
        cat_bufs = []
        v = a = None
        nin = len(arch_in)
        for i, layers in enumerate(arch_in):
            chp, ich = skip_cols[nin - 1 - i]
            Ho, Lo = Hh, L
            for layer in layers:
                if layer["kind"] == "res" and layer["down"]:
                    Ho, Lo = Hh // 2, L // 4
            ops.cur_sid = 0
            vcat = self._alloc(N * F * Ho * Ho, chp + ich, stats=True, unit=F * Ho * Ho)
            ops.cur_sid = 1
            acat = self._alloc(N * Lo, chp + ich, stats=True, unit=Lo)
            ops.cur_sid = 0
            cat_bufs.append((vcat, acat))
            ov, oa = vcat[:, chp:], acat[:, chp:]
            for j, layer in enumerate(layers):
                last = j == len(layers) - 1
                tv, ta = (ov, oa) if last else (None, None)
                if layer["kind"] == "init":
                    C0 = layer["cout"]
                    p = layer["prefix"]
                    s1 = self._alloc(N * F * Hh * Hh, C0)
                    ops.stem_conv(self.x_video, self._edge_w(p + ".video_conv.video_conv_spatial.weight"),
                                  self._f32(p + ".video_conv.video_conv_spatial.bias"), s1, N, F, self.Cv_in, Hh, Hh,
                                  ops.TAPS_SPATIAL)
                    nv = tv if tv is not None else self._alloc(N * F * Hh * Hh, C0, stats=True, unit=F * Hh * Hh)
                    ops.conv_gemm(s1, self._gemm_w(p + ".video_conv.video_conv_temporal.weight"),
                                  self._f32(p + ".video_conv.video_conv_temporal.bias"), **self._temporal(Hh), out=nv,
                                  **self._stats_kw(nv))
                    self._release(s1)
                    ops.record_sync(1, 0)
                    film_joined = True
                    ops.cur_sid = 1
                    na = ta if ta is not None else self._alloc(N * L, C0)
                    ops.stem_conv(self.x_audio, self._edge_w(p + ".audio_conv.audio_conv.weight"),
                                  self._f32(p + ".audio_conv.audio_conv.bias"), na, N, 1, self.Ca_in, 1, L,
                                  [(0, 0, -1), (0, 0, 0), (0, 0, 1)])
                    ops.cur_sid = 0
                elif layer["kind"] == "res":
                    if not film_joined:
                        ops.record_sync(1, 0)
                        film_joined = True
                    nv, na, Hh, L = self._res(v, a, layer, Hh, L, tv, ta)
                else:
                    nv, na = self._cross(v, a, layer, Hh, L, tv, ta)
                if j > 0:
                    self._release(v, a)
                v, a = nv, na

        def run_block(layers, v, a, Hh, L, ov, oa, own_input):
            for j, layer in enumerate(layers):
                last = j == len(layers) - 1
                tv, ta = (ov, oa) if last else (None, None)
                if layer["kind"] == "res":
                    nv, na, Hh, L = self._res(v, a, layer, Hh, L, tv, ta)
                else:
                    nv, na = self._cross(v, a, layer, Hh, L, tv, ta)
                if j > 0 or own_input:
                    self._release(v, a)
                v, a = nv, na
            return v, a, Hh, L

        vcat, acat = cat_bufs[-1]
        chp, _ = skip_cols[0]
        v, a, Hh, L = run_block(arch_mid, v, a, Hh, L, vcat[:, :chp], acat[:, :chp], own_input=False)

        for k, layers in enumerate(arch_out):
            vcat, acat = cat_bufs[nin - 1 - k]
            if k + 1 < len(arch_out):
                nvcat, nacat = cat_bufs[nin - 2 - k]
                chn, _ = skip_cols[k + 1]
                ov, oa = nvcat[:, :chn], nacat[:, :chn]
            else:
                ov = oa = None
            v, a, Hh, L = run_block(layers, vcat, acat, Hh, L, ov, oa, own_input=False)
            self._release(vcat, acat)

        ops.cur_sid = 0
        gh = Geom.per_sample(N, F * Hh * Hh)
        hw = self._edge_w("video_out.2.video_conv.weight")
        hv = None
        if ops.head_gemm_ok(v, hw, gh):
            ga, gb = self._gn_affine(v, "video_out.0", gh, None)
            NO = hw.shape[0] * hw.shape[2]
            P = self._alloc(NO, v.shape[0], torch.float32)
            ops.head_gemm(v, ga, gb, gh, True, self._packed("head_gemm", "video_out.2.video_conv.weight", lambda: ops.head_gemm_pack(hw)), P, NO)
            ops.head_gather(P, self._f32("video_out.2.video_conv.bias"), self.out_video, N, F, Hh, Hh, hw.shape[2], ops.TAPS_3D)
            self._release(ga, gb, P)
        else:
            hv = self._gn(v, "video_out.0", gh, act=True)
            ops.head_conv(hv, hw, self._f32("video_out.2.video_conv.bias"), self.out_video, N, F, Hh, Hh, ops.TAPS_3D)
        ops.cur_sid = 1
        ha = self._gn(a, "audio_out.0", Geom.per_sample(N, L), act=True)
        ops.head_conv(ha, self._edge_w("audio_out.2.audio_conv.weight"), self._f32("audio_out.2.audio_conv.bias"),
                      self.out_audio, N, 1, 1, L, [(0, 0, -1), (0, 0, 0), (0, 0, 1)])
        ops.cur_sid = 0
        self._release(hv, ha, v, a)
        if self._deferred:
            ops.record_sync(1, 0)
            self._release(*self._deferred)
            self._deferred = []

    def set_inputs(self, video, audio, timesteps, shifts):
        N = self.N
        if tuple(video.shape) != tuple(self.x_video.shape) or tuple(audio.shape) != tuple(self.x_audio.shape):
            raise H.MMDError(f"input shapes {tuple(video.shape)}/{tuple(audio.shape)} do not match the model's "
                             f"{tuple(self.x_video.shape)}/{tuple(self.x_audio.shape)}")
        if video.data_ptr() != self.x_video.data_ptr():
            self.x_video.copy_(video)
        if audio.data_ptr() != self.x_audio.data_ptr():
            self.x_audio.copy_(audio)
        use_f32 = timesteps.dtype.is_floating_point
        tgt = self.t_f32 if use_f32 else self.t_i64
        if timesteps.data_ptr() != tgt.data_ptr():
            tgt.copy_(timesteps)
        self.set_shifts(shifts)
        return use_f32

    def set_shifts(self, shifts):
        if self.nshift:
            if len(shifts) != self.nshift:
                raise H.MMDError(f"expected {self.nshift} window shifts, got {len(shifts)}")
            host = self._shift_up.host()
            for i, s in enumerate(shifts):
# ... 61 lines not shown
```

mm-diffusion_amd/mm_diffusion/ops.py:

```python
import math
import os

import torch

from . import _hip as H

GN_EPS = 1e-5

_recorder = None
_keep = None


class recording:
    def __init__(self, plan, keep=None):
        self.plan, self.keep = plan, keep

    def __enter__(self):
        global _recorder, _keep
        self._prev, _recorder = (_recorder, _keep), self.plan
        _keep = self.keep
        return self.plan

    def __exit__(self, *a):
        global _recorder, _keep
        _recorder, _keep = self._prev


def alloc(*shape, dtype, device):
    t = torch.empty(*shape, dtype=dtype, device=device)
    if _keep is not None and _recorder is not None:
        _keep.append(t)
    return t


cur_sid = 0
cur_tag = ""


def _dispatch(name, *args, meta=None):
    if _recorder is not None:
        _recorder.append((getattr(H.lib(), name), args, name, meta or (name, 0, 0), cur_sid, cur_tag))
    else:
        H.call(name, *args, H.stream_handle())


def record_sync(src, dst):
    import ctypes
    ev = ctypes.c_void_p()
    H.call("mmd_event_create", ctypes.byref(ev))
    _recorder.append((None, (src, dst, ev), "sync", None, -1, ""))


_SKIP_SID = int(os.environ["MMD_SKIP_SID"]) if os.environ.get("MMD_SKIP_SID", "") in ("0", "1") else None
_SKIP_WAIT = os.environ.get("MMD_SKIP_WAIT", "")
if _SKIP_SID is not None or _SKIP_WAIT:
    import warnings
    warnings.warn("MMD_SKIP_SID / MMD_SKIP_WAIT are set: replayed plans DROP a launch chain or cross-stream waits - timing experiments only, "
                  "every output of this process is wrong", RuntimeWarning)
_TIMING_ONLY_OK = os.environ.get("MMD_TIMING_ONLY", "") == "1"


def run_plan(plan, stream, aux_stream=None):
    lib = H.lib()
    if (_SKIP_SID is not None or _SKIP_WAIT) and not _TIMING_ONLY_OK:
        raise H.MMDError("MMD_SKIP_SID / MMD_SKIP_WAIT (timing experiments: they drop launches / waits from every replayed plan) need "
                         "MMD_TIMING_ONLY=1 as well - refusing to replay a plan whose outputs would be silently wrong")
    streams = (stream, aux_stream if aux_stream is not None else stream)
    for fn, args, name, _, sid, _tag in plan:
        if fn is None:
            if aux_stream is not None:
                src, dst, ev = args
                if _SKIP_WAIT and _SKIP_WAIT == f"{src}{dst}":
                    continue
                if lib.mmd_event_record(ev, streams[src]) or lib.mmd_stream_wait_event(streams[dst], ev):
                    raise H.MMDError(f"sync failed: {lib.mmd_last_error().decode()}")
            continue
        if _SKIP_SID is not None and sid == _SKIP_SID:
            continue
        rc = fn(*args, streams[sid])
        if rc != 0:
            raise H.MMDError(f"{name} failed ({rc}): {lib.mmd_last_error().decode()}")


class Geom:
    __slots__ = ("S", "Tn", "inner", "outer_stride", "inner_stride", "tstride")

    def __init__(self, S, Tn, inner=1, outer_stride=None, inner_stride=1, tstride=1):
        self.S, self.Tn, self.inner = int(S), int(Tn), int(inner)
        self.outer_stride = int(Tn if outer_stride is None else outer_stride)
        self.inner_stride, self.tstride = int(inner_stride), int(tstride)

    @staticmethod
    def per_sample(N, rows_per_sample):
        return Geom(N, rows_per_sample, 1, rows_per_sample, 1, 1)

    @staticmethod
    def spatial(N, F, HW):
        return Geom(N * F, HW, 1, HW, 1, 1)

    @staticmethod
    def temporal(N, F, HW):
        return Geom(N * HW, F, HW, F * HW, 1, HW)

    def args(self):
        return (self.S, self.Tn, self.inner, self.outer_stride, self.inner_stride, self.tstride)


def _chk2d(t):
    if t.dim() != 2 or t.stride(1) != 1:
        raise H.MMDError(f"expected a [rows, C] tensor with unit channel stride, got {tuple(t.shape)} strides {t.stride()}")
    H.require_cuda(t)


def gn_workspace_bytes(x, geom: Geom):
    return max(8, int(H.lib().mmd_gn_workspace_bytes(H.dt_of(x), x.shape[1], geom.S, geom.Tn)))


def gn_workspace(x, geom: Geom):
    return alloc(gn_workspace_bytes(x, geom) // 8, dtype=torch.float64, device=x.device)


def gn_stats(x, gamma, beta, geom: Geom, film=None, a=None, b=None, ws=None, mr=None):
    _chk2d(x)
    C = x.shape[1]
    a = alloc(geom.S, C, dtype=torch.float32, device=x.device) if a is None else a
    b = alloc(geom.S, C, dtype=torch.float32, device=x.device) if b is None else b
    ws = gn_workspace(x, geom) if ws is None else ws
    _dispatch("mmd_gn_stats", H.dt_of(x), x.data_ptr(), x.stride(0), C, *geom.args(), gamma.data_ptr(), beta.data_ptr(),
           H.ptr(film), 0 if film is None else film.stride(0), GN_EPS, a.data_ptr(), b.data_ptr(), H.ptr(mr), ws.data_ptr(),
           meta=(f"gn_stats[S={geom.S},Tn={geom.Tn},C={C}]", 0, geom.S * geom.Tn * C * x.element_size()))
    return a, b


def gn_finalize_stats(rec, gamma, beta, geom: Geom, film=None, a=None, b=None, mr=None):
    C = rec.shape[1] * 4
    if C % 128:
        raise H.MMDError("gn_finalize_stats: the normalised channels must be a multiple of 128 (groups of whole quads)")
    if geom.inner != 1 or geom.tstride != 1 or geom.outer_stride != geom.Tn or geom.Tn % 64 or rec.shape[0] * 64 != geom.S * geom.Tn:
        raise H.MMDError("gn_finalize_stats: needs contiguous slices that are multiples of 64 rows")
    a = alloc(geom.S, C, dtype=torch.float32, device=rec.device) if a is None else a
    b = alloc(geom.S, C, dtype=torch.float32, device=rec.device) if b is None else b
    _dispatch("mmd_gn_finalize_stats", rec.data_ptr(), rec.stride(0) // 2, C, geom.S, geom.Tn, gamma.data_ptr(), beta.data_ptr(),
              H.ptr(film), 0 if film is None else film.stride(0), GN_EPS, a.data_ptr(), b.data_ptr(), H.ptr(mr),
              meta=(f"gn_finalize_stats[S={geom.S},Tn={geom.Tn},C={C}]", 0, rec.shape[0] * C * 8))
    return a, b


def gn_apply(x, a, b, geom: Geom, act=True, out=None):
    _chk2d(x)
    out = alloc(x.shape, dtype=x.dtype, device=x.device) if out is None else out
    _chk2d(out)
    _dispatch("mmd_gn_apply", H.dt_of(x), x.data_ptr(), x.stride(0), out.data_ptr(), out.stride(0), x.shape[0], x.shape[1],
           *geom.args(), a.data_ptr(), b.data_ptr(), 1 if act else 0,
           meta=("gn_apply", 0, 2 * x.shape[0] * x.shape[1] * x.element_size()))
    return out


def zero(t):
    H.require_cuda(t)
    _dispatch("mmd_zero", t.data_ptr(), t.numel() * t.element_size(), meta=("zero", 0, t.numel() * t.element_size()))
    return t


def gn_small_ok(x, geom: Geom):
    return geom.Tn <= 16 and x.shape[1] % 128 == 0 and x.shape[1] // (8 if x.element_size() == 2 else 4) <= 256


def gn_small(x, gamma, beta, geom: Geom, act=False, out=None):
    _chk2d(x)
    out = alloc(x.shape, dtype=x.dtype, device=x.device) if out is None else out
    _chk2d(out)
    _dispatch("mmd_gn_small", H.dt_of(x), x.data_ptr(), x.stride(0), out.data_ptr(), out.stride(0), x.shape[1], *geom.args(), gamma.data_ptr(),
              beta.data_ptr(), GN_EPS, 1 if act else 0, meta=(f"gn_small[S={geom.S},Tn={geom.Tn},C={x.shape[1]}]", 0, 2 * x.shape[0] * x.shape[1] * x.element_size()))
    return out


_GN_GROUP = os.environ.get("MMD_GN_GROUP", "1") != "0"


def gn_group_ok(x, geom: Geom):
    C = x.shape[1]
    return _GN_GROUP and C % 128 == 0 and C <= 2048 and geom.Tn * (C // 128) <= 4096 and x.stride(0) % 4 == 0


def gn_group(x, gamma, beta, geom: Geom, film=None, a=None, b=None, out=None, act=False, mr=None):
    _chk2d(x)
    C = x.shape[1]
    if out is None and a is None:
        a = alloc(geom.S, C, dtype=torch.float32, device=x.device)
        b = alloc(geom.S, C, dtype=torch.float32, device=x.device)
    if out is not None:
        _chk2d(out)
    _dispatch("mmd_gn_group", H.dt_of(x), x.data_ptr(), x.stride(0), H.ptr(out), 0 if out is None else out.stride(0), C, *geom.args(),
              gamma.data_ptr(), beta.data_ptr(), H.ptr(film), 0 if film is None else film.stride(0), GN_EPS, 1 if act else 0,
              H.ptr(a), H.ptr(b), H.ptr(mr),
              meta=(f"gn_group[S={geom.S},Tn={geom.Tn},C={C}]", 0, (1 if out is None else 2) * geom.S * geom.Tn * C * x.element_size()))
    return (a, b) if out is None else out


def add_rowbias(x, e, rows_per_sample):
    _chk2d(x)
    _dispatch("mmd_add_rowbias", H.dt_of(x), x.data_ptr(), x.stride(0), x.shape[0], x.shape[1], rows_per_sample,
           e.data_ptr(), e.stride(0))
    return x


def colsum_slices(dy, out, rows_per_sample):
    _chk2d(dy)
    S = dy.shape[0] // rows_per_sample
    _dispatch("mmd_colsum_slices", H.dt_of(dy), dy.data_ptr(), dy.stride(0), S, rows_per_sample, dy.shape[1], out.data_ptr(), out.stride(0))
    return out


TAPS_1 = [(0, 0, 0)]
TAPS_SPATIAL = [(0, dh, dw) for dh in (-1, 0, 1) for dw in (-1, 0, 1)]
TAPS_TEMPORAL = [(df, 0, 0) for df in (-1, 0, 1)]
TAPS_TEMPORAL_D1 = [(0, df, 0) for df in (-1, 0, 1)]
TAPS_3D = [(df, dh, dw) for df in (-1, 0, 1) for dh in (-1, 0, 1) for dw in (-1, 0, 1)]


def taps_audio(dilation):
    return [(-dilation, 0, 0), (0, 0, 0), (dilation, 0, 0)]


AUTOTUNE = True
_tile_cache = {}


# ... 44 lines not shown
            best, best_ms = tile, t_min
    for e in ev:
        H.lib().mmd_event_destroy(e)
    for t, keep in saved:
        t.copy_(keep)
    _tile_cache[key] = best
    return best


_HALO_MODE = os.environ.get("MMD_GEMM_HALO", "pin")
HALO_CANDIDATE = _HALO_MODE == "1"


def halo_tile_ok(x, taps, dims):
    M, Cin = x.shape
    return (len(taps) > 1 and all(t[0] == 0 and abs(t[1]) <= 1 and abs(t[2]) <= 1 for t in taps) and dims[1] % 8 == 0
            and dims[2] % 16 == 0 and dims[0] * dims[1] * dims[2] == M and Cin % (128 // x.element_size()) == 0)


_HALO16 = os.environ.get("MMD_HALO16", "1") != "0"


def halo_tile_code(x, taps, dims):
    return 133 if (_HALO16 and x.dtype == torch.bfloat16 and len(taps) == 9 and dims[1] % 16 == 0 and dims[2] % 16 == 0
                   and x.shape[1] >= 256 and tuple(tuple(t) for t in taps) == tuple(TAPS_SPATIAL)) else 130


def _stats_args(stats, M, Cout):
    if (stats.dtype != torch.float32 or Cout % 4 or tuple(stats.shape) != (M // 64, Cout // 4, 2) or M % 64 or stats.stride(1) != 2
            or stats.stride(2) != 1):
        raise H.MMDError(f"GEMM output statistics: expected an fp32 [M/64, Cout/4, 2] view, got {tuple(stats.shape)} strides {stats.stride()}")
    return stats.data_ptr(), stats.stride(0) // 2


_HALO_MIN_PIXELS = int(os.environ.get("MMD_HALO_MIN_PIXELS", "1024"))


def halo_tile_pinned(x, taps, dims):
    return (_HALO_MODE == "pin" and x.dtype == torch.bfloat16 and len(taps) == 9 and dims[1] * dims[2] >= _HALO_MIN_PIXELS
            and halo_tile_ok(x, taps, dims))


_STRIP_MODE = os.environ.get("MMD_GEMM_STRIP", "pin")


def strip_tile_ok(x, Cout, taps=TAPS_1, stats=None, geom=None, base=False):
    M, Cin = x.shape
    K = len(taps) * Cin
    if x.dtype != torch.bfloat16 or K not in (128, 256, 384, 512) or Cin % 64:
        return False
    if len(taps) == 1 and tuple(taps[0]) != (0, 0, 0):
        return False
    rf = 2 if K <= 256 else 1
    if Cout % (32 * rf) or Cout > 2048 or (stats is not None and M % 64):
        return False
    if base and (len(taps) != 1 or K == 512 or (stats is not None and rf != 2)):
        return False
    if geom is not None and not (len(taps) == 1 and geom.inner == 1 and geom.tstride == 1 and geom.outer_stride == geom.Tn
                                 and geom.Tn >= 128 * rf and geom.S * geom.Tn == M):
        return False
    return True


def strip_tile_pinned(x, Cout, taps=TAPS_1, stats=None, geom=None):
    if _STRIP_MODE == "0":
        return False
    return strip_tile_ok(x, Cout, taps, stats, geom, base=_STRIP_MODE == "base")


def _tile_name(tile):
    return {129: "128glds", 130: "128halo", 131: "strip", 132: "128ring", 133: "256halo"}.get(tile, tile)


_RING_MODE = os.environ.get("MMD_GEMM_RING", "1")


def ring_tile_candidate(x, Cout, ntaps):
    M, Cin = x.shape
    kstep = 128 // x.element_size()
    return (_RING_MODE != "0" and Cin % kstep == 0 and (Cin * ntaps) // kstep >= 4
            and ((M + 127) // 128) * ((Cout + 127) // 128) <= 384)


def conv_gemm(x, w, bias, taps=TAPS_1, dims=(1, 1, 1), residual=None, out=None, tile=0, stats=None):
    _chk2d(x)
    M, Cin = x.shape
    Cout = w.shape[0]
    if w.dtype != x.dtype or w.shape[1] != len(taps) * Cin or not w.is_contiguous():
        raise H.MMDError(f"conv_gemm: weight {tuple(w.shape)} {w.dtype} does not match input {tuple(x.shape)} {x.dtype} x {len(taps)} taps")
    out = alloc(M, Cout, dtype=x.dtype, device=x.device) if out is None else out
    _chk2d(out)
    arr, nt = H.taps_array(taps)
    es = x.element_size()
    base = (H.dt_of(x), x.data_ptr(), x.stride(0), w.data_ptr(), H.ptr(bias), H.ptr(residual),
            0 if residual is None else residual.stride(0), out.data_ptr(), out.stride(0), M, Cout, Cin, nt, arr,
            int(dims[0]), int(dims[1]), int(dims[2]))
    if tile == 0 and stats is None and halo_tile_pinned(x, taps, dims):
        tile = halo_tile_code(x, taps, dims)
    if tile == 0 and strip_tile_pinned(x, Cout, taps, stats):
        tile = 131
    if tile == 0:
        cands = (128, 129) if stats is not None else (64, 128, 129) + ((130,) if HALO_CANDIDATE and halo_tile_ok(x, taps, dims) else ())
        if ring_tile_candidate(x, Cout, nt):
            cands = cands + (132,)
        tile = _pick_tile((es, M, Cin, nt, Cout, residual is not None, False, tuple(dims) if 130 in cands else None),
                          lambda t: H.call("mmd_conv_gemm", *base, t, H.stream_handle()), M, Cout, cands, out=out, scratch=(x, residual))
    flops = 2 * M * Cout * Cin * nt
    nbytes = es * (M * Cin + M * Cout * (2 if residual is not None else 1) + Cout * Cin * nt) + 4 * Cout
    label = f"conv_gemm<{'bf16' if es == 2 else 'f32'},{_tile_name(tile)}>[M={M},K={Cin * nt},N={Cout}]"
    if stats is not None:
        _dispatch("mmd_conv_gemm_stats", *base, tile, *_stats_args(stats, M, Cout), meta=(label, flops, nbytes))
    else:
        _dispatch("mmd_conv_gemm", *base, tile, meta=(label, flops, nbytes))
    return out


_STRIP_BLOCKS_RULE = int(os.environ.get("MMD_STRIP_BLOCKS_RULE", "448"))


def strip_column_split(M, K, Cout):
    rf, cc = (2, 64) if K <= 256 else (1, 32)
    rowblocks, nch, n = -(-M // (128 * rf)), Cout // cc, 1
    for d in range(1, min(nch, 16) + 1):
        if nch % d == 0:
            n = d
            if rowblocks * d >= _STRIP_BLOCKS_RULE:
                break
    return n


def gn_fusable(geom: Geom, Cin, Cout, x=None, stats=None, act=False):
    if x is not None and strip_tile_pinned(x, Cout, stats=stats):
        if not strip_tile_pinned(x, Cout, stats=stats, geom=geom):
            return False
        return not (act and strip_column_split(x.shape[0], Cin, Cout) > 2)
    return (geom.inner == 1 and geom.tstride == 1 and geom.outer_stride == geom.Tn and geom.Tn >= 128 and Cin <= 256
            and (Cout + 127) // 128 <= 2)


def gn_conv1x1(x, a, b, geom: Geom, act, w, bias, residual=None, out=None, tile=0, stats=None):
    _chk2d(x)
    M, Cin = x.shape
    Cout = w.shape[0]
    if w.dtype != x.dtype or w.shape[1] != Cin or not w.is_contiguous():
        raise H.MMDError(f"gn_conv1x1: weight {tuple(w.shape)} {w.dtype} does not match input {tuple(x.shape)} {x.dtype}")
    out = alloc(M, Cout, dtype=x.dtype, device=x.device) if out is None else out
    _chk2d(out)
    es = x.element_size()
    tiled_ok = (geom.inner == 1 and geom.tstride == 1 and geom.outer_stride == geom.Tn and geom.Tn >= 128 and Cin <= 256
                and (Cout + 127) // 128 <= 2)
    strip_ok = strip_tile_ok(x, Cout, stats=stats, geom=geom)
    if not ((tile == 131 and strip_ok) or (tile in (64, 128) and tiled_ok) or (tile == 0 and (tiled_ok or strip_ok))):
        raise H.MMDError("gn_conv1x1: needs contiguous slices of >= 128 rows, Cin <= 256 (use gn_apply + conv_gemm otherwise)")
    base = (H.dt_of(x), x.data_ptr(), x.stride(0), a.data_ptr(), b.data_ptr(), 1 if act else 0, geom.S, geom.Tn,
            w.data_ptr(), H.ptr(bias), H.ptr(residual),
            0 if residual is None else residual.stride(0), out.data_ptr(), out.stride(0), M, Cout, Cin)
    if tile == 0 and strip_tile_pinned(x, Cout, stats=stats, geom=geom):
        tile = 131
    if tile == 0 and not tiled_ok:
        raise H.MMDError("gn_conv1x1: the row-strip kernel is switched off (MMD_GEMM_STRIP) and the tiled loader cannot take this launch")
    if tile == 0:
        tile = _pick_tile((es, M, Cin, 1, Cout, residual is not None, True),
                          lambda t: H.call("mmd_gn_conv1x1", *base, t, H.stream_handle()), M, Cout,
                          candidates=(128,) if stats is not None else (64, 128), out=out, scratch=(x, residual, a, b))
    nbytes = es * (M * Cin + M * Cout * (2 if residual is not None else 1) + Cout * Cin) + 4 * Cout
    meta = (f"gn_conv1x1<{'bf16' if es == 2 else 'f32'},{_tile_name(tile)}>[M={M},K={Cin},N={Cout}]", 2 * M * Cout * Cin, nbytes)
    if stats is not None:
        _dispatch("mmd_gn_conv1x1_stats", *base, tile, *_stats_args(stats, M, Cout), meta=meta)
    else:
        _dispatch("mmd_gn_conv1x1", *base, tile, meta=meta)
    return out


_HALO_GN = os.environ.get("MMD_HALO_GN", "1") != "0"


def halo_gn_ok(x, taps, dims, geom: Geom):
    return (_HALO_GN and halo_tile_pinned(x, taps, dims) and geom.inner == 1 and geom.tstride == 1 and geom.outer_stride == geom.Tn
            and geom.S * geom.Tn == x.shape[0] and geom.Tn % (dims[1] * dims[2]) == 0)


def gn_conv_gemm(x, a, b, geom: Geom, act, w, bias, taps, dims, residual=None, out=None, tile=0):
    _chk2d(x)
    M, Cin = x.shape
    Cout = w.shape[0]
    if w.dtype != x.dtype or w.shape[1] != len(taps) * Cin or not w.is_contiguous():
        raise H.MMDError(f"gn_conv_gemm: weight {tuple(w.shape)} {w.dtype} does not match input {tuple(x.shape)} {x.dtype} x {len(taps)} taps")
    if not (halo_tile_ok(x, taps, dims) and len(taps) == 9 and x.dtype == torch.bfloat16 and geom.S * geom.Tn == M
            and geom.inner == 1 and geom.tstride == 1 and geom.outer_stride == geom.Tn and geom.Tn % (dims[1] * dims[2]) == 0):
        raise H.MMDError("gn_conv_gemm: needs a bf16 3x3 conv tile 130 accepts and contiguous slices of whole frames")
    out = alloc(M, Cout, dtype=x.dtype, device=x.device) if out is None else out
    _chk2d(out)
    arr, nt = H.taps_array(taps)
    es = x.element_size()
    flops = 2 * M * Cout * Cin * nt
    nbytes = es * (M * Cin + M * Cout * (2 if residual is not None else 1) + Cout * Cin * nt) + 4 * Cout
    _dispatch("mmd_gn_conv_gemm", H.dt_of(x), x.data_ptr(), x.stride(0), a.data_ptr(), b.data_ptr(), 1 if act else 0, geom.S, geom.Tn,
              w.data_ptr(), H.ptr(bias), H.ptr(residual), 0 if residual is None else residual.stride(0), out.data_ptr(), out.stride(0),
              M, Cout, Cin, nt, arr, int(dims[0]), int(dims[1]), int(dims[2]), tile or halo_tile_code(x, taps, dims),
              meta=(f"gn_conv_gemm<bf16,{_tile_name(tile or halo_tile_code(x, taps, dims))}>[M={M},K={Cin * nt},N={Cout}]", flops, nbytes))
    return out


_VCONV_FUSED = os.environ.get("MMD_VCONV_FUSED", "1") != "0"


def vconv_shape_ok(x, Cout, N, F, Hh, Ww):
    return (x.dtype == torch.bfloat16 and F == 16 and Cout == 128 and x.shape[1] % 32 == 0 and Hh % 4 == 0 and Ww % 4 == 0
            and x.shape[0] == N * F * Hh * Ww and (16 * Hh * Ww * x.stride(0) + x.shape[1]) * 2 < 2 ** 31)


def _ranges_overlap(x, y):
    x0, y0 = x.data_ptr(), y.data_ptr()
    x1 = x0 + ((x.shape[0] - 1) * x.stride(0) + x.shape[1]) * x.element_size()
    y1 = y0 + ((y.shape[0] - 1) * y.stride(0) + y.shape[1]) * y.element_size()
    return not (x1 <= y0 or y1 <= x0)


def vconv_fused_ok(x, Cout, N, F, Hh, Ww, out=None):
    return _VCONV_FUSED and vconv_shape_ok(x, Cout, N, F, Hh, Ww) and (out is None or not _ranges_overlap(x, out))


def vconv_pack(ws, wt):
    H.require_cuda(ws, wt)
    Cout, Cin = ws.shape[0], ws.shape[1] // 9
    if ws.dtype != torch.bfloat16 or wt.dtype != torch.bfloat16 or tuple(wt.shape) != (Cout, 3 * Cout) or not ws.is_contiguous() or not wt.is_contiguous():
        raise H.MMDError(f"vconv_pack: expected contiguous bf16 [Cout, 9 Cin] / [Cout, 3 Cout], got {tuple(ws.shape)} / {tuple(wt.shape)}")
    out = torch.empty(H.lib().mmd_vconv2d1d_weight_bytes(Cin) // 2, dtype=torch.bfloat16, device=ws.device)
    H.call("mmd_vconv2d1d_pack", ws.data_ptr(), wt.data_ptr(), out.data_ptr(), Cin, Cout, H.stream_handle())
    return out


def vconv2d1d(x, wf, bias_s, bias_t, N, F, Hh, Ww, a=None, b=None, geom=None, act=True, out=None, stats=None):
    _chk2d(x)
    M, Cin = x.shape
    Cout = 128
    if not vconv_shape_ok(x, Cout, N, F, Hh, Ww):
        raise H.MMDError(f"vconv2d1d: unsupported launch (x {tuple(x.shape)} {x.dtype}, N={N} F={F} H={Hh} W={Ww})")
    if (a is None) != (b is None) or (a is not None and (geom is None or geom.inner != 1 or geom.tstride != 1 or geom.outer_stride != geom.Tn
                                                         or geom.S * geom.Tn != M or geom.Tn % (F * Hh * Ww))):
        raise H.MMDError("vconv2d1d: the fused input norm needs contiguous slices of whole samples")
    out = alloc(M, Cout, dtype=x.dtype, device=x.device) if out is None else out
    _chk2d(out)
    if _ranges_overlap(x, out) or tuple(out.shape) != (M, Cout) or out.dtype != x.dtype:
        raise H.MMDError("vconv2d1d: the output must be a bf16 [M, 128] tensor whose address range does not overlap the input's (the C side "
                         "compares whole ranges: column slices of one buffer count as overlapping)")
    if wf.numel() * wf.element_size() != H.lib().mmd_vconv2d1d_weight_bytes(Cin):
        raise H.MMDError("vconv2d1d: the weight image does not match Cin (pack it with vconv_pack)")
    sp, sld = (None, 0) if stats is None else _stats_args(stats, M, Cout)
    flops = 2 * M * Cout * (9 * Cin + 3 * Cout)
# ... 478 lines not shown
```

Measured before the change: 350.5 pair-steps/s.

## Fold GroupNorm finalize into producing row-strip GEMM via last-block counters

Adds fold variants of the row-strip conv1x1/conv_gemm kernels. They write the per-row-block GroupNorm partial statistics atomically, and the last block per slice, found with an atomic counter, reduces them in double precision and writes the affine a/b coefficients. In the recorded graph, the model rewrites the producer entry to the fold variant and skips the separate gn_finalize_stats launch. This removes one small kernel launch and its dependency per eligible norm. In exchange it adds a tail reduction with a barrier inside the GEMM, device-scope atomics, and extra build-time asm checks.

```diff
diff --git a/include/mmd.h b/include/mmd.h
--- a/include/mmd.h
+++ b/include/mmd.h
@@ -70,6 +70,27 @@
 int mmd_gn_conv1x1_stats(int dtype, const void* A, int64_t lda, const float* gn_a, const float* gn_b, int act, int S,
                          int64_t rows_per_slice, const void* W, const float* bias, const void* R, int64_t ldr, void* Y, int64_t ldy,
                          int M, int Cout, int Cin, int tile, float* stats, int64_t stats_ld, void* stream);
+
+typedef struct MmdGnFold {
+  const float* rec;
+  int64_t rec_ld;
+  int C, S, Tn;
+  const float* gamma;
+  const float* beta;
+  const float* film;
+  int64_t film_ld;
+  float eps;
+  float* a_out;
+  float* b_out;
+  float* mr_out;
+  unsigned int* counters;
+} MmdGnFold;
+int mmd_conv_gemm_stats_fold(int dtype, const void* A, int64_t lda, const void* W, const float* bias, const void* R, int64_t ldr,
+                             void* Y, int64_t ldy, int M, int Cout, int Cin, int ntaps, const int* taps, int D0, int D1, int D2, int tile,
+                             float* stats, int64_t stats_ld, const MmdGnFold* fold, void* stream);
+int mmd_gn_conv1x1_stats_fold(int dtype, const void* A, int64_t lda, const float* gn_a, const float* gn_b, int act, int S,
+                              int64_t rows_per_slice, const void* W, const float* bias, const void* R, int64_t ldr, void* Y, int64_t ldy,
+                              int M, int Cout, int Cin, int tile, float* stats, int64_t stats_ld, const MmdGnFold* fold, void* stream);
 
 int mmd_gn_conv_gemm(int dtype, const void* A, int64_t lda, const float* gn_a, const float* gn_b, int act, int S,
                      int64_t rows_per_slice, const void* W, const float* bias, const void* R, int64_t ldr, void* Y, int64_t ldy,
diff --git a/mm-diffusion_amd/build.py b/mm-diffusion_amd/build.py
--- a/mm-diffusion_amd/build.py
+++ b/mm-diffusion_amd/build.py
@@ -73,6 +73,23 @@
         raise RuntimeError("build check: conv1x1_strip_res_kernel: %d kernels checked, %d violations%s" % (n, len(bad), (": " + bad[0]) if bad else ""))
 
 
+def _check_gn_fold_asm(obj):
+    import importlib.util
+    tools = os.path.join(os.path.dirname(HERE), "tools")
+    spec = importlib.util.spec_from_file_location("gn_fold_asm_check", os.path.join(tools, "gn_fold_asm_check.py"))
+    chk = importlib.util.module_from_spec(spec)
+    spec.loader.exec_module(chk)
+    import strip_asm_check
+    strip_asm_check.LLVM = _llvm_bin()
+    asm = strip_asm_check.disassemble(obj)
+    n, bad = chk.check(asm)
+    nr, badr = chk.check_residual_registers(asm)
+    bad += badr
+    if n == 0 or nr == 0 or bad:
+        raise RuntimeError("build check: row-strip fold instances: %d kernels checked (%d with a residual), %d violations%s" %
+                           (n, nr, len(bad), (": " + bad[0]) if bad else ""))
+
+
 def build(force=False, verbose=True):
     if not force and not _stale():
         return OUT
@@ -99,6 +116,7 @@
         subprocess.check_call(cmd)
         _check_no_packed_f32(tmp)
         _check_strip_asm(os.path.join(HERE, "lib", "mmd_gemm.o"))
+        _check_gn_fold_asm(os.path.join(HERE, "lib", "mmd_gemm.o"))
         os.replace(tmp, OUT)
     finally:
         if os.path.exists(tmp):
diff --git a/mm-diffusion_amd/csrc/mmd_common.h b/mm-diffusion_amd/csrc/mmd_common.h
--- a/mm-diffusion_amd/csrc/mmd_common.h
+++ b/mm-diffusion_amd/csrc/mmd_common.h
@@ -110,6 +110,109 @@
   return dpp_add<0x142, 0xa>(v);
 }
 
+#define GN_GROUPS 32
+#define GN_FOLD_REC 128
+typedef __attribute__((address_space(1))) unsigned int gu32;
+typedef __attribute__((address_space(1))) uint64_t gu64;
+
+__device__ __forceinline__ void gn_rec_affine(double sa, double sb, double cnt, float eps, float gv, float bv0, bool film, float fsc,
+                                              float fsh, float& mean_f, float& rstd_f, float& av, float& bv) {
+  const double mean = sa / cnt;
+  double var = sb / cnt - mean * mean;
+  if (var < 0.0) var = 0.0;
+  mean_f = (float)mean;
+  rstd_f = (float)(1.0 / sqrt(var + (double)eps));
+  av = rstd_f * gv;
+  bv = bv0 - mean_f * av;
+  if (film) {
+    const float sc = 1.f + fsc;
+    av *= sc;
+    bv = bv * sc + fsh;
+  }
+}
+
+__device__ __forceinline__ void gn_fold_slice(const MmdGnFold& f, int s) {
+  const int lane = threadIdx.x & 63, w = threadIdx.x >> 6;
+  const int cpg = f.C / GN_GROUPS, qpg = cpg / 4, nrec = f.Tn / 64, total = nrec * qpg;
+  const int nv = (total + 63) >> 6;
+  const char* rbase = (const char*)(f.rec + (int64_t)s * nrec * f.rec_ld * 2);
+  const uint32_t ld8 = (uint32_t)f.rec_ld * 8u;
+  uint32_t off[2];
+#pragma unroll
+  for (int u = 0; u < 2; ++u) {
+    const int kk = min(64 * u + lane, total - 1);
+    const int r = kk / qpg, cq = kk - r * qpg;
+    off[u] = (uint32_t)r * ld8 + (uint32_t)cq * 8u;
+  }
+  uint64_t v[8][2];
+#pragma unroll
+  for (int j = 0; j < 8; ++j)
+#pragma unroll
+    for (int u = 0; u < 2; ++u)
+      v[j][u] = __hip_atomic_load((const gu64*)(rbase + (uint32_t)((w + 4 * j) * qpg * 8) + off[u]), __ATOMIC_RELAXED,
+                                  __HIP_MEMORY_SCOPE_AGENT);
+  const int cl = min(lane, cpg - 1);
+  float gv[8], bv0[8], fsc[8], fsh[8];
+#pragma unroll
+  for (int j = 0; j < 8; ++j) {
+    const int c = (w + 4 * j) * cpg + cl;
+    gv[j] = f.gamma[c];
+    bv0[j] = f.beta[c];
+    fsc[j] = fsh[j] = 0.f;
+    if (f.film) {
+      fsc[j] = f.film[(int64_t)s * f.film_ld + c];
+      fsh[j] = f.film[(int64_t)s * f.film_ld + f.C + c];
+    }
+  }
+  const double cnt = (double)f.Tn * (double)cpg;
+#pragma unroll
+  for (int j = 0; j < 8; ++j) {
+    double sa[4] = {0.0, 0.0, 0.0, 0.0}, sb[4] = {0.0, 0.0, 0.0, 0.0};
+#pragma unroll
+    for (int u = 0; u < 2; ++u) {
+      if (u < nv) {
+        const bool ok = 64 * u + lane < total;
+        const double x = ok ? (double)__uint_as_float((uint32_t)v[j][u]) + 0.0 : 0.0;
+        const double y = ok ? (double)__uint_as_float((uint32_t)(v[j][u] >> 32)) + 0.0 : 0.0;
+        sa[u] = wave_sum_d(x);
+        sb[u] = wave_sum_d(y);
+      }
+    }
+    const double ta = (sa[0] + sa[1]) + (sa[2] + sa[3]), tb = (sb[0] + sb[1]) + (sb[2] + sb[3]);
+    float mean_f, rstd_f, av, bv;
+    gn_rec_affine(ta, tb, cnt, f.eps, gv[j], bv0[j], f.film != nullptr, fsc[j], fsh[j], mean_f, rstd_f, av, bv);
+    const int gi = w + 4 * j;
+    if (f.mr_out && lane == 0) {
+      f.mr_out[((int64_t)s * GN_GROUPS + gi) * 2] = mean_f;
+      f.mr_out[((int64_t)s * GN_GROUPS + gi) * 2 + 1] = rstd_f;
+    }
+    if (lane < cpg) {
+      f.a_out[(int64_t)s * f.C + gi * cpg + lane] = av;
+      f.b_out[(int64_t)s * f.C + gi * cpg + lane] = bv;
+    }
+  }
+}
+
+__device__ __forceinline__ void gn_fold_tail(const MmdGnFold& f, int r0, int r1, int BR, int nsplit, int* s_flag) {
+  asm volatile("s_waitcnt vmcnt(0) lgkmcnt(0)" ::: "memory");
+  __builtin_amdgcn_s_barrier();
+  asm volatile("" ::: "memory");
+  const int s0 = r0 / f.Tn, s1 = (r1 - 1) / f.Tn;
+  if (threadIdx.x == 0) {
+    for (int s = s0; s <= s1; ++s) {
+      const unsigned want = (unsigned)nsplit * (unsigned)(((s + 1) * f.Tn - 1) / BR - (s * f.Tn) / BR + 1);
+      const unsigned old = __hip_atomic_fetch_add((gu32*)(f.counters + s), 1u, __ATOMIC_RELAXED, __HIP_MEMORY_SCOPE_AGENT);
+      const bool last = old + 1 == want;
+      if (last) __hip_atomic_store((gu32*)(f.counters + s), 0u, __ATOMIC_RELAXED, __HIP_MEMORY_SCOPE_AGENT);
+      s_flag[s - s0] = last;
+    }
+  }
+  asm volatile("s_waitcnt lgkmcnt(0)" ::: "memory");
+  __builtin_amdgcn_s_barrier();
+  asm volatile("" ::: "memory");
+  for (int s = s0; s <= s1; ++s)
+    if (__builtin_amdgcn_readfirstlane(s_flag[s - s0])) gn_fold_slice(f, s);
+}
 
 static inline int cdiv(int64_t a, int64_t b) { return (int)((a + b - 1) / b); }
 
diff --git a/mm-diffusion_amd/csrc/mmd_gemm.hip b/mm-diffusion_amd/csrc/mmd_gemm.hip
--- a/mm-diffusion_amd/csrc/mmd_gemm.hip
+++ b/mm-diffusion_amd/csrc/mmd_gemm.hip
@@ -1249,8 +1249,17 @@
                    : "=v"(rf[0]), "=v"(rf[1]), "=v"(rf[2]), "=v"(rf[3]), "=v"(rf[4]), "=v"(rf[5]), "=v"(rf[6]), "=v"(rf[7]) : "n"(n));  \
   } while (0)
 __host__ __device__ constexpr int wait_imm(int vm) { return (vm & 15) | ((vm >> 4) << 14) | 0x0070; }
+template <int STM>
+__device__ __forceinline__ void strip_rec_store(float* d, float sum, float sq) {
+  if constexpr (STM == 2) {
+    __hip_atomic_store((gu64*)d, ((uint64_t)__float_as_uint(sq) << 32) | __float_as_uint(sum), __ATOMIC_RELAXED, __HIP_MEMORY_SCOPE_AGENT);
+  } else {
+    d[0] = sum;
+    d[1] = sq;
+  }
+}
 template <int KS, int RF, int CC, int GNM, int STM, bool HR>
-__device__ __forceinline__ void conv1x1_strip_body(const ConvGemmParams& p, const int nsplit) {
+__device__ __forceinline__ void conv1x1_strip_body(const ConvGemmParams& p, const int nsplit, const MmdGnFold& fold) {
   constexpr int K = 64 * KS;
   constexpr int NCG = 4 * KS;
   constexpr int BR = 128 * RF;
@@ -1513,7 +1522,7 @@
       for (int t = 0; t < NSTEP; ++t) epi_step(s_, ac, kp, t, dma_between, last);
     };
     auto commit = [&](int s_, float (&kp)[2][2]) __attribute__((always_inline)) {
-      if (STM == 1 && wave_ok && (RF == 2 || (wave & 1) == 0) && (l31 >> 1) == 8) {
+      if (STM != 0 && wave_ok && (RF == 2 || (wave & 1) == 0) && (l31 >> 1) == 8) {
         const int a = s_ % NA, par = (s_ / NA) & 1;
 #pragma unroll
         for (int j2 = 0; j2 < 2; ++j2) {
@@ -1525,8 +1534,7 @@
             o0 = o[0];
             o1 = o[1];
           }
-          d[0] = kp[j2][0] + o0;
-          d[1] = kp[j2][1] + o1;
+          strip_rec_store<STM>(d, kp[j2][0] + o0, kp[j2][1] + o1);
         }
       }
     };
@@ -1556,7 +1564,7 @@
     auto tail = [&](f32x16 (&ac)[RF], float (&kp)[2][2], float (&kq)[2][2]) __attribute__((always_inline)) {
       epi(NS - 1, ac, kp, false, true);
       if (RF == 2) commit(NS - 1, kp);
-      if (RF == 1 && STM == 1) {
+      if (RF == 1 && STM != 0) {
         __builtin_amdgcn_s_waitcnt(wait_imm(63));
         __builtin_amdgcn_s_barrier();
         if (NS >= 2) commit(NS - 2, kq);
@@ -1638,7 +1646,7 @@
             }
           }
         }
-        if (STM == 1) {
+        if (STM != 0) {
           const float t0 = halfwave_total(u[0]), t1 = halfwave_total(u[1]), t2 = halfwave_total(u[2]), t3 = halfwave_total(u[3]);
           const float msum = (l31 & 1) ? t1 : t0, msq = (l31 & 1) ? t3 : t2;
           if (RF == 1) {
@@ -1651,8 +1659,7 @@
             srec[j2][1] = msq;
           } else if (wave_ok && (l31 >> 1) == 8) {
             float* d = p.stats + (rec * p.stats_ld + (col >> 2) + (l31 & 1)) * 2;
-            d[0] = msum;
-            d[1] = msq;
+            strip_rec_store<STM>(d, msum, msq);
           }
         }
       }
@@ -1666,30 +1673,39 @@
       for (int f = 0; f < RF; ++f)
         *(u32x4*)(p.Y + (int64_t)(cbase + ci * CC + (NA - 1) * 32 + 16 * j2) * 2 + yoff[f]) = outv[f][j2];
       if (RF == 1) {
-        if (STM == 1 && wave_ok && (wave & 1) == 0 && (l31 >> 1) == 8) {
+        if (STM != 0 && wave_ok && (wave & 1) == 0 && (l31 >> 1) == 8) {
           const float* o = sRec + ((((ci & 1) * 4 + wave + 1) * (NA * 2) + (NA - 1) * 2 + j2) * 2 + half) * 4 + (l31 & 1) * 2;
           float* d = p.stats + (rec * p.stats_ld + (col >> 2) + (l31 & 1)) * 2;
-          d[0] = srec[j2][0] + o[0];
-          d[1] = srec[j2][1] + o[1];
+          strip_rec_store<STM>(d, srec[j2][0] + o[0], srec[j2][1] + o[1]);
         }
       }
     }
   }
   }
+  if constexpr (STM == 2) gn_fold_tail(fold, m0, min(m0 + BR, p.M), BR, nsplit, (int*)smem);
 }
 
 #define STRIP_LAUNCH_BOUNDS __launch_bounds__(256, (KS <= 2 ? (RF == 1 ? 4 : 3) : 2))
 template <int KS, int RF, int CC, int GNM, int STM>
 __global__ STRIP_LAUNCH_BOUNDS void conv1x1_strip_kernel(const ConvGemmParams p, const int nsplit) {
-  conv1x1_strip_body<KS, RF, CC, GNM, STM, false>(p, nsplit);
+  conv1x1_strip_body<KS, RF, CC, GNM, STM, false>(p, nsplit, MmdGnFold{});
 }
 template <int KS, int RF, int CC, int GNM, int STM>
 __global__ STRIP_LAUNCH_BOUNDS __attribute__((amdgpu_num_vgpr(248))) void conv1x1_strip_res_kernel(const ConvGemmParams p, const int nsplit) {
-  conv1x1_strip_body<KS, RF, CC, GNM, STM, true>(p, nsplit);
+  conv1x1_strip_body<KS, RF, CC, GNM, STM, true>(p, nsplit, MmdGnFold{});
+}
+template <int KS, int RF, int CC, int GNM>
+__global__ STRIP_LAUNCH_BOUNDS void conv1x1_strip_fold_kernel(const ConvGemmParams p, const int nsplit, const MmdGnFold fold) {
+  conv1x1_strip_body<KS, RF, CC, GNM, 2, false>(p, nsplit, fold);
+}
+template <int KS, int RF, int CC, int GNM>
+__global__ STRIP_LAUNCH_BOUNDS __attribute__((amdgpu_num_vgpr(248))) void conv1x1_strip_fold_res_kernel(const ConvGemmParams p, const int nsplit,
+                                                                                                  const MmdGnFold fold) {
+  conv1x1_strip_body<KS, RF, CC, GNM, 2, true>(p, nsplit, fold);
 }
 
 template <int KS, int RF, int CC, int GNM, int STM, bool HR>
-static int launch_conv1x1_strip_res(const ConvGemmParams& p, hipStream_t st) {
+static int launch_conv1x1_strip_res(const ConvGemmParams& p, hipStream_t st, const MmdGnFold& fold) {
   constexpr int BR = 128 * RF, STAGE_B = KS * CC * 128;
   const int rowblocks = cdiv(p.M, BR), nch = p.Cout / CC;
   static const int want_blocks = [] {
@@ -1711,33 +1727,45 @@
   static bool attr_done[MMD_MAX_DEVICES] = {};
   bool& attr_set = attr_done[mmd_device_slot()];
   if (!attr_set) {
-    const void* kfn = HR ? (const void*)conv1x1_strip_res_kernel<KS, RF, CC, GNM, STM> : (const void*)conv1x1_strip_kernel<KS, RF, CC, GNM, STM>;
+    const void* kfn;
+    if constexpr (STM == 2) kfn = HR ? (const void*)conv1x1_strip_fold_res_kernel<KS, RF, CC, GNM> : (const void*)conv1x1_strip_fold_kernel<KS, RF, CC, GNM>;
+    else kfn = HR ? (const void*)conv1x1_strip_res_kernel<KS, RF, CC, GNM, STM> : (const void*)conv1x1_strip_kernel<KS, RF, CC, GNM, STM>;
     hipError_t e = hipFuncSetAttribute(kfn, hipFuncAttributeMaxDynamicSharedMemorySize, (int)lds_max);
     if (e != hipSuccess) return mmd_set_error(MMD_ERR_LAUNCH, "conv1x1_strip: set LDS attr: %s", hipGetErrorString(e));
     attr_set = true;
   }
-  if (HR) hipLaunchKernelGGL((conv1x1_strip_res_kernel<KS, RF, CC, GNM, STM>), dim3(rowblocks * nsplit), dim3(256), lds, st, p, nsplit);
-  else hipLaunchKernelGGL((conv1x1_strip_kernel<KS, RF, CC, GNM, STM>), dim3(rowblocks * nsplit), dim3(256), lds, st, p, nsplit);
+  if constexpr (STM == 2) {
+    if (HR) hipLaunchKernelGGL((conv1x1_strip_fold_res_kernel<KS, RF, CC, GNM>), dim3(rowblocks * nsplit), dim3(256), lds, st, p, nsplit, fold);
+    else hipLaunchKernelGGL((conv1x1_strip_fold_kernel<KS, RF, CC, GNM>), dim3(rowblocks * nsplit), dim3(256), lds, st, p, nsplit, fold);
+  } else {
+    if (HR) hipLaunchKernelGGL((conv1x1_strip_res_kernel<KS, RF, CC, GNM, STM>), dim3(rowblocks * nsplit), dim3(256), lds, st, p, nsplit);
+    else hipLaunchKernelGGL((conv1x1_strip_kernel<KS, RF, CC, GNM, STM>), dim3(rowblocks * nsplit), dim3(256), lds, st, p, nsplit);
+  }
   return mmd_check_launch("conv1x1_strip");
 }
 
 template <int KS, int RF, int CC, int GNM, int STM>
-static int launch_conv1x1_strip_mode(const ConvGemmParams& p, hipStream_t st) {
-  return p.R ? launch_conv1x1_strip_res<KS, RF, CC, GNM, STM, true>(p, st) : launch_conv1x1_strip_res<KS, RF, CC, GNM, STM, false>(p, st);
+static int launch_conv1x1_strip_mode(const ConvGemmParams& p, hipStream_t st, const MmdGnFold& fold) {
+  return p.R ? launch_conv1x1_strip_res<KS, RF, CC, GNM, STM, true>(p, st, fold) : launch_conv1x1_strip_res<KS, RF, CC, GNM, STM, false>(p, st, fold);
 }
 
 template <int KS, int RF, int CC, int STM>
-static int launch_conv1x1_strip_st(const ConvGemmParams& p, hipStream_t st) {
-  if (!p.gn_a) return launch_conv1x1_strip_mode<KS, RF, CC, 0, STM>(p, st);
-  return p.gn_act ? launch_conv1x1_strip_mode<KS, RF, CC, 2, STM>(p, st) : launch_conv1x1_strip_mode<KS, RF, CC, 1, STM>(p, st);
+static int launch_conv1x1_strip_st(const ConvGemmParams& p, hipStream_t st, const MmdGnFold& fold) {
+  if (!p.gn_a) return launch_conv1x1_strip_mode<KS, RF, CC, 0, STM>(p, st, fold);
+  return p.gn_act ? launch_conv1x1_strip_mode<KS, RF, CC, 2, STM>(p, st, fold) : launch_conv1x1_strip_mode<KS, RF, CC, 1, STM>(p, st, fold);
 }
 
 template <int KS, int RF, int CC>
-static int launch_conv1x1_strip(const ConvGemmParams& p, hipStream_t st) {
-  return p.stats ? launch_conv1x1_strip_st<KS, RF, CC, 1>(p, st) : launch_conv1x1_strip_st<KS, RF, CC, 0>(p, st);
-}
-
-static int dispatch_conv1x1_strip(const ConvGemmParams& p, hipStream_t st) {
+static int launch_conv1x1_strip(const ConvGemmParams& p, hipStream_t st, const MmdGnFold* fold) {
+  static const MmdGnFold none = {};
+  if (fold) {
+    if constexpr (KS >= 4) return launch_conv1x1_strip_st<KS, RF, CC, 2>(p, st, *fold);
+    else return mmd_set_error(MMD_ERR_UNSUPPORTED, "conv_gemm fold: the row-strip kernel folds a norm only at K = ntaps * Cin >= 256");
+  }
+  return p.stats ? launch_conv1x1_strip_st<KS, RF, CC, 1>(p, st, none) : launch_conv1x1_strip_st<KS, RF, CC, 0>(p, st, none);
+}
+
+static int dispatch_conv1x1_strip(const ConvGemmParams& p, hipStream_t st, const MmdGnFold* fold) {
   const int K = p.Cin * p.ntaps;
   const int rf = K <= 256 ? 2 : 1, cc = K <= 256 ? 64 : 32;
   if ((K != 128 && K != 256 && K != 384 && K != 512) || p.Cin % 64 != 0 || p.Cout % cc != 0 ||
@@ -1747,12 +1775,12 @@
                          "fused GroupNorm only for 1x1 convs with slices of >= %d rows (got Cin=%d ntaps=%d Cout=%d)", cc, 128 * rf, p.Cin, p.ntaps, p.Cout);
   if (K == 128) {
     static const bool rf1 = [] { const char* e = getenv("MMD_STRIP_K128_RF1"); return !(e && e[0] == '0'); }();
-    if (rf1 && p.gn_a && p.gn_rows >= 16384 && p.ntaps == 1 && p.Cout % 32 == 0) return launch_conv1x1_strip<2, 1, 32>(p, st);
-    return launch_conv1x1_strip<2, 2, 64>(p, st);
-  }
-  if (K == 256) return launch_conv1x1_strip<4, 2, 64>(p, st);
-  if (K == 384) return launch_conv1x1_strip<6, 1, 32>(p, st);
-  return launch_conv1x1_strip<8, 1, 32>(p, st);
+    if (rf1 && p.gn_a && p.gn_rows >= 16384 && p.ntaps == 1 && p.Cout % 32 == 0) return launch_conv1x1_strip<2, 1, 32>(p, st, fold);
+    return launch_conv1x1_strip<2, 2, 64>(p, st, fold);
+  }
+  if (K == 256) return launch_conv1x1_strip<4, 2, 64>(p, st, fold);
+  if (K == 384) return launch_conv1x1_strip<6, 1, 32>(p, st, fold);
+  return launch_conv1x1_strip<8, 1, 32>(p, st, fold);
 }
 
 template <typename T, bool GN>
@@ -1896,7 +1924,7 @@
 static int conv_gemm_impl(int dtype, const void* A, int64_t lda, const void* W, const float* bias, const void* R, int64_t ldr,
                           void* Y, int64_t ldy, int M, int Cout, int Cin, int ntaps, const int* taps, int D0, int D1, int D2,
                           int tile, const float* gn_a, const float* gn_b, int gn_act, int gn_S, int64_t gn_rows, float* stats,
-                          int64_t stats_ld, void* stream) {
+                          int64_t stats_ld, void* stream, const MmdGnFold* fold = nullptr) {
   const int epv = dtype == MMD_BF16 ? 8 : 4;
   MMD_REQUIRE(dtype == MMD_BF16 || dtype == MMD_F32, "conv_gemm: bad dtype %d", dtype);
   MMD_REQUIRE(A && W && Y && M > 0 && Cout > 0 && Cin > 0, "conv_gemm: null/empty argument");
@@ -1925,7 +1953,19 @@
                   ((tile == 131 || tile == 133) && dtype == MMD_BF16),
               "conv_gemm: tile must be 0, 64, 128, 129 (128 direct-to-LDS), 130 (halo-tile 3x3), 131 (row strip, bf16 1x1 convs) or 132 (129 with a "
               "four-slot ring for launches of few tiles)");
-  if (tile == 131) return dispatch_conv1x1_strip(p, st);
+  if (fold) {
+    const intptr_t off = (intptr_t)fold->rec - (intptr_t)stats;
+    const int64_t q0 = off / 8;
+    MMD_REQUIRE(tile == 131 && stats && fold->rec && fold->gamma && fold->beta && fold->a_out && fold->b_out && fold->counters,
+                "conv_gemm fold: needs the row-strip tile (131), output statistics and non-null records / affine / outputs / counters");
+    MMD_REQUIRE(fold->C > 0 && fold->C % (4 * GN_GROUPS) == 0 && fold->C <= 2048 && fold->S > 0 && fold->Tn > 0 && fold->Tn % 64 == 0 &&
+                    (int64_t)fold->S * fold->Tn == M && (int64_t)(fold->Tn / 64) * (fold->C / (4 * GN_GROUPS)) <= GN_FOLD_REC,
+                "conv_gemm fold: C %% 128 == 0, C <= 2048, S slices of Tn %% 64 == 0 rows covering M and <= 128 records per (slice, group) "
+                "(got C=%d S=%d Tn=%d M=%d)", fold->C, fold->S, fold->Tn, M);
+    MMD_REQUIRE(fold->rec_ld == stats_ld && off >= 0 && off % 8 == 0 && q0 + fold->C / 4 <= Cout / 4,
+                "conv_gemm fold: the norm's records must be a column range of this launch's records (same row stride)");
+  }
+  if (tile == 131) return dispatch_conv1x1_strip(p, st, fold);
   return dtype == MMD_BF16 ? dispatch_conv_gemm<__bf16>(p, tile, st) : dispatch_conv_gemm<float>(p, tile, st);
 }
 
@@ -1960,6 +2000,24 @@
   MMD_REQUIRE(gn_a && gn_b && stats, "gn_conv1x1_stats: null GroupNorm affine / statistics buffer");
   return conv_gemm_impl(dtype, A, lda, W, bias, R, ldr, Y, ldy, M, Cout, Cin, 1, tap0, 1, 1, 1, tile, gn_a, gn_b, act, S,
                         rows_per_slice, stats, stats_ld, stream);
+}
+
+extern "C" int mmd_conv_gemm_stats_fold(int dtype, const void* A, int64_t lda, const void* W, const float* bias, const void* R, int64_t ldr,
+                                        void* Y, int64_t ldy, int M, int Cout, int Cin, int ntaps, const int* taps, int D0, int D1, int D2,
+                                        int tile, float* stats, int64_t stats_ld, const MmdGnFold* fold, void* stream) {
+  MMD_REQUIRE(stats && fold, "conv_gemm_stats_fold: null statistics buffer / fold descriptor");
+  return conv_gemm_impl(dtype, A, lda, W, bias, R, ldr, Y, ldy, M, Cout, Cin, ntaps, taps, D0, D1, D2, tile, nullptr, nullptr, 0, 0,
+                        0, stats, stats_ld, stream, fold);
+}
+
+extern "C" int mmd_gn_conv1x1_stats_fold(int dtype, const void* A, int64_t lda, const float* gn_a, const float* gn_b, int act, int S,
+                                         int64_t rows_per_slice, const void* W, const float* bias, const void* R, int64_t ldr, void* Y,
+                                         int64_t ldy, int M, int Cout, int Cin, int tile, float* stats, int64_t stats_ld,
+                                         const MmdGnFold* fold, void* stream) {
+  static const int tap0[3] = {0, 0, 0};
+  MMD_REQUIRE(gn_a && gn_b && stats && fold, "gn_conv1x1_stats_fold: null GroupNorm affine / statistics buffer / fold descriptor");
+  return conv_gemm_impl(dtype, A, lda, W, bias, R, ldr, Y, ldy, M, Cout, Cin, 1, tap0, 1, 1, 1, tile, gn_a, gn_b, act, S,
+                        rows_per_slice, stats, stats_ld, stream, fold);
 }
 
 extern "C" int mmd_gn_conv_gemm(int dtype, const void* A, int64_t lda, const float* gn_a, const float* gn_b, int act, int S,
diff --git a/mm-diffusion_amd/csrc/mmd_norm.hip b/mm-diffusion_amd/csrc/mmd_norm.hip
--- a/mm-diffusion_amd/csrc/mmd_norm.hip
+++ b/mm-diffusion_amd/csrc/mmd_norm.hip
@@ -1,6 +1,5 @@
 #include "mmd_common.h"
 
-#define GN_GROUPS 32
 typedef __attribute__((ext_vector_type(2))) double f64x2;
 
 struct SliceGeom {
@@ -461,21 +460,11 @@
   __syncthreads();
   if (tid < cpg) {
     const double sa = (s_a[0] + s_a[1]) + (s_a[2] + s_a[3]), sb = (s_b[0] + s_b[1]) + (s_b[2] + s_b[3]);
-    const double cnt = (double)Tn * (double)cpg;
-    const double mean = sa / cnt;
-    double var = sb / cnt - mean * mean;
-    if (var < 0.0) var = 0.0;
-    const float mean_f = (float)mean, rstd_f = (float)(1.0 / sqrt(var + (double)eps));
+    float mean_f, rstd_f, av, bv;
+    gn_rec_affine(sa, sb, (double)Tn * (double)cpg, eps, gv, bv0, film != nullptr, fsc, fsh, mean_f, rstd_f, av, bv);
     if (mr_out && tid == 0) {
       mr_out[((int64_t)s * GN_GROUPS + gi) * 2] = mean_f;
       mr_out[((int64_t)s * GN_GROUPS + gi) * 2 + 1] = rstd_f;
-    }
-    float av = rstd_f * gv;
-    float bv = bv0 - mean_f * av;
-    if (film) {
-      const float sc = 1.f + fsc;
-      av *= sc;
-      bv = bv * sc + fsh;
     }
     a_out[(int64_t)s * C + c] = av;
     b_out[(int64_t)s * C + c] = bv;
diff --git a/mm-diffusion_amd/mm_diffusion/_hip.py b/mm-diffusion_amd/mm_diffusion/_hip.py
--- a/mm-diffusion_amd/mm_diffusion/_hip.py
+++ b/mm-diffusion_amd/mm_diffusion/_hip.py
@@ -11,6 +11,11 @@
 _lib = None
 
 i32, i64, f32, vp = C.c_int, C.c_int64, C.c_float, C.c_void_p
+
+
+class MmdGnFold(C.Structure):
+    _fields_ = [("rec", vp), ("rec_ld", i64), ("C", i32), ("S", i32), ("Tn", i32), ("gamma", vp), ("beta", vp), ("film", vp),
+                ("film_ld", i64), ("eps", f32), ("a_out", vp), ("b_out", vp), ("mr_out", vp), ("counters", vp)]
 
 
 _PROTOS = {
@@ -42,6 +47,10 @@
     "mmd_gn_conv1x1": (i32, [i32, vp, i64, vp, vp, i32, i32, i64, vp, vp, vp, i64, vp, i64, i32, i32, i32, i32, vp]),
     "mmd_conv_gemm_stats": (i32, [i32, vp, i64, vp, vp, vp, i64, vp, i64, i32, i32, i32, i32, C.POINTER(i32), i32, i32, i32, i32, vp, i64, vp]),
     "mmd_gn_conv1x1_stats": (i32, [i32, vp, i64, vp, vp, i32, i32, i64, vp, vp, vp, i64, vp, i64, i32, i32, i32, i32, vp, i64, vp]),
+    "mmd_conv_gemm_stats_fold": (i32, [i32, vp, i64, vp, vp, vp, i64, vp, i64, i32, i32, i32, i32, C.POINTER(i32), i32, i32, i32, i32, vp, i64,
+                                       C.POINTER(MmdGnFold), vp]),
+    "mmd_gn_conv1x1_stats_fold": (i32, [i32, vp, i64, vp, vp, i32, i32, i64, vp, vp, vp, i64, vp, i64, i32, i32, i32, i32, vp, i64,
+                                        C.POINTER(MmdGnFold), vp]),
     "mmd_gn_conv_gemm": (i32, [i32, vp, i64, vp, vp, i32, i32, i64, vp, vp, vp, i64, vp, i64, i32, i32, i32, i32, C.POINTER(i32), i32, i32, i32, i32, vp]),
     "mmd_tconv_weight_bytes": (i64, [i32, i32]),
     "mmd_tconv_pack": (i32, [vp, vp, i32, i32, vp]),
diff --git a/mm-diffusion_amd/mm_diffusion/engine.py b/mm-diffusion_amd/mm_diffusion/engine.py
--- a/mm-diffusion_amd/mm_diffusion/engine.py
+++ b/mm-diffusion_amd/mm_diffusion/engine.py
@@ -12,6 +12,11 @@
 _UP_LOWRES = os.environ.get("MMD_UP_LOWRES", "1") != "0"
 _CROSS_SERIAL = os.environ.get("MMD_CROSS_SERIAL", "1") != "0"
 _RESAMPLE_STATS = os.environ.get("MMD_RESAMPLE_STATS", "1") != "0"
+
+
+def fold_eligible(bf16, producers, covered, entry_name, tile, k_ok, same_stream, rec_bytes, film_ready):
+    return (bf16 and producers == 1 and covered and entry_name in ops.FOLD_ENTRIES and tile == 131 and k_ok and same_stream
+            and rec_bytes <= ops.FOLD_MAX_REC_BYTES and film_ready)
 
 
 class _Pool:
@@ -60,6 +65,8 @@
         mode = os.environ.get("MMD_GN_EPILOGUE", "1")
         self.rec_enabled = mode == "2" or (mode != "0" and dtype == torch.bfloat16)
         self._recs = {}
+        self._film_at = {}
+        self.n_folded = 0
         self._gn_small = os.environ.get("MMD_GN_SMALL", "1") != "0"
         self._vconv_fused = self._tattn_fused = self._tconv = self._aconv = dtype == torch.bfloat16
         self._deferred = []
@@ -113,7 +120,10 @@
             return None
         ent["perm_unit"] = max(ent.get("perm_unit", 0), perm_unit)
         ent["cover"].append((c0, c0 + out.shape[1]))
-        return ent["view"][:, c0 // 4:(c0 + out.shape[1]) // 4, :]
+        view = ent["view"][:, c0 // 4:(c0 + out.shape[1]) // 4, :]
+        if ops._recorder is not None:
+            ent.setdefault("prods", []).append((c0, c0 + out.shape[1], ops._recorder, len(ops._recorder), view.data_ptr()))
+        return view
 
     def _has_stats(self, out):
         return self._rec_slice(out)[0] is not None
@@ -144,6 +154,25 @@
             pos = max(pos, hi)
         return ent["view"][:, c0 // 4:need // 4, :] if pos >= need else None
 
+    def _fold_producer(self, x, geom, film):
+        plan = ops._recorder
+        ent, c0 = self._rec_slice(x)
+        lo, hi = c0, c0 + x.shape[1]
+        prods = [p for p in ent.get("prods", ()) if p[0] < hi and p[1] > lo]
+        if plan is None or len(prods) != 1 or prods[0][2] is not plan or prods[0][3] >= len(plan):
+            return None
+        plo, phi, _, idx, rec_ptr = prods[0]
+        fn, args, name, meta, sid, tag = plan[idx]
+        if name in ops.FOLD_ENTRIES and args[ops.FOLD_TILE_ARG + 1] != rec_ptr:
+            return None
+        film_at = self._film_at.get(sid)
+        film_ready = film is None or (film_at is not None and idx >= film_at)
+        ok = fold_eligible(self.dtype == torch.bfloat16, len(prods), plo <= lo and phi >= hi, name,
+                           args[ops.FOLD_TILE_ARG] if name in ops.FOLD_ENTRIES else None, ops.FOLD_MIN_K <= ops.fold_k(name, args),
+                           sid == ops.cur_sid,
+                           ops.fold_rec_bytes(geom, x.shape[1]), film_ready)
+        return idx if ok else None
+
     def _static(self, shape, dtype):
         t = torch.zeros(shape, dtype=dtype, device=self.device)
         self.keep.append(t)
@@ -195,7 +224,15 @@
         b = self._alloc(geom.S, C, torch.float32)
         gamma, beta = self._f32(prefix + ".GroupNorm.weight"), self._f32(prefix + ".GroupNorm.bias")
         rec = self._rec_ready(x, geom)
-        if rec is not None:
+        idx = None if rec is None else self._fold_producer(x, geom, film)
+        if idx is not None:
+            self._release(a, b)
+            a, b = self._static((geom.S, C), torch.float32), self._static((geom.S, C), torch.float32)
+            desc, _, _ = ops.gn_fold_desc(rec, gamma, beta, geom, self._static((geom.S,), torch.int32), film=film, a=a, b=b)
+            self.keep.append(desc)
+            ops._recorder[idx] = ops.fold_entry(ops._recorder[idx], desc)
+            self.n_folded += 1
+        elif rec is not None:
             ops.gn_finalize_stats(rec, gamma, beta, geom, film=film, a=a, b=b)
         elif ops.gn_group_ok(x, geom):
             ops.gn_group(x, gamma, beta, geom, film=film, a=a, b=b)
@@ -495,10 +532,12 @@
         ops.temb(t_tensor, mc, self._f32("time_embed.0.weight"), self._f32("time_embed.0.bias"),
                  self._f32("time_embed.2.weight"), self._f32("time_embed.2.bias"), self.emb_silu)
         ops.linear(self.emb_silu, self.emb_W, self.emb_b, self.emb_all)
+        self._film_at[ops.cur_sid] = len(ops._recorder)
         ops.cur_sid = 0
         film_joined = not _EMB_ON_AUDIO_STREAM
         if not _EMB_ON_AUDIO_STREAM:
             ops.record_sync(0, 1)
+            self._film_at[1] = len(ops._recorder)
 
         skip_cols = []
         ch = arch_mid[-1]["cout"]
@@ -540,6 +579,7 @@
                                   **self._stats_kw(nv))
                     self._release(s1)
                     ops.record_sync(1, 0)
+                    self._film_at[0] = len(ops._recorder)
                     film_joined = True
                     ops.cur_sid = 1
                     na = ta if ta is not None else self._alloc(N * L, C0)
@@ -550,6 +590,7 @@
                 elif layer["kind"] == "res":
                     if not film_joined:
                         ops.record_sync(1, 0)
+                        self._film_at[0] = len(ops._recorder)
                         film_joined = True
                     nv, na, Hh, L = self._res(v, a, layer, Hh, L, tv, ta)
                 else:
diff --git a/mm-diffusion_amd/mm_diffusion/ops.py b/mm-diffusion_amd/mm_diffusion/ops.py
--- a/mm-diffusion_amd/mm_diffusion/ops.py
+++ b/mm-diffusion_amd/mm_diffusion/ops.py
@@ -1,3 +1,4 @@
+import ctypes
 import math
 import os
 
@@ -144,6 +145,40 @@
               H.ptr(film), 0 if film is None else film.stride(0), GN_EPS, a.data_ptr(), b.data_ptr(), H.ptr(mr),
               meta=(f"gn_finalize_stats[S={geom.S},Tn={geom.Tn},C={C}]", 0, rec.shape[0] * C * 8))
     return a, b
+
+
+FOLD_MAX_REC_BYTES = 32768
+FOLD_ENTRIES = {"mmd_conv_gemm_stats": "mmd_conv_gemm_stats_fold", "mmd_gn_conv1x1_stats": "mmd_gn_conv1x1_stats_fold"}
+FOLD_TILE_ARG = 17
+FOLD_MIN_K = 256
+
+
+def fold_k(name, args):
+    return args[11] * args[12] if name == "mmd_conv_gemm_stats" else args[16] if name == "mmd_gn_conv1x1_stats" else 0
+
+
+def fold_rec_bytes(geom: Geom, C):
+    return (geom.Tn // 64) * (C // 4) * 8
+
+
+def gn_fold_desc(rec, gamma, beta, geom: Geom, counters, film=None, a=None, b=None, mr=None):
+    C = rec.shape[1] * 4
+    if C % 128 or geom.inner != 1 or geom.tstride != 1 or geom.outer_stride != geom.Tn or geom.Tn % 64 or rec.shape[0] * 64 != geom.S * geom.Tn:
+        raise H.MMDError("gn_fold: needs C % 128 == 0 and contiguous slices that are multiples of 64 rows")
+    if counters.dtype != torch.int32 or counters.numel() < geom.S or not counters.is_contiguous():
+        raise H.MMDError(f"gn_fold: needs {geom.S} contiguous int32 counters")
+    a = alloc(geom.S, C, dtype=torch.float32, device=rec.device) if a is None else a
+    b = alloc(geom.S, C, dtype=torch.float32, device=rec.device) if b is None else b
+    d = H.MmdGnFold(rec.data_ptr(), rec.stride(0) // 2, C, geom.S, geom.Tn, gamma.data_ptr(), beta.data_ptr(), H.ptr(film),
+                    0 if film is None else film.stride(0), GN_EPS, a.data_ptr(), b.data_ptr(), H.ptr(mr), counters.data_ptr())
+    return d, a, b
+
+
+def fold_entry(entry, desc):
+    fn, args, name, meta, sid, tag = entry
+    fname = FOLD_ENTRIES[name]
+    label, flops, nbytes = meta
+    return (getattr(H.lib(), fname), tuple(args) + (ctypes.pointer(desc),), fname, (label + "+gn_fold", flops, nbytes), sid, tag)
 
 
 def gn_apply(x, a, b, geom: Geom, act=True, out=None):
@@ -354,7 +389,7 @@
             and ((M + 127) // 128) * ((Cout + 127) // 128) <= 384)
 
 
-def conv_gemm(x, w, bias, taps=TAPS_1, dims=(1, 1, 1), residual=None, out=None, tile=0, stats=None):
+def conv_gemm(x, w, bias, taps=TAPS_1, dims=(1, 1, 1), residual=None, out=None, tile=0, stats=None, fold=None):
     _chk2d(x)
     M, Cin = x.shape
     Cout = w.shape[0]
@@ -380,7 +415,9 @@
     flops = 2 * M * Cout * Cin * nt
     nbytes = es * (M * Cin + M * Cout * (2 if residual is not None else 1) + Cout * Cin * nt) + 4 * Cout
     label = f"conv_gemm<{'bf16' if es == 2 else 'f32'},{_tile_name(tile)}>[M={M},K={Cin * nt},N={Cout}]"
-    if stats is not None:
+    if fold is not None:
+        _dispatch("mmd_conv_gemm_stats_fold", *base, tile, *_stats_args(stats, M, Cout), ctypes.pointer(fold), meta=(label, flops, nbytes))
+    elif stats is not None:
         _dispatch("mmd_conv_gemm_stats", *base, tile, *_stats_args(stats, M, Cout), meta=(label, flops, nbytes))
     else:
         _dispatch("mmd_conv_gemm", *base, tile, meta=(label, flops, nbytes))
@@ -410,7 +447,7 @@
             and (Cout + 127) // 128 <= 2)
 
 
-def gn_conv1x1(x, a, b, geom: Geom, act, w, bias, residual=None, out=None, tile=0, stats=None):
+def gn_conv1x1(x, a, b, geom: Geom, act, w, bias, residual=None, out=None, tile=0, stats=None, fold=None):
     _chk2d(x)
     M, Cin = x.shape
     Cout = w.shape[0]
@@ -437,7 +474,9 @@
                           candidates=(128,) if stats is not None else (64, 128), out=out, scratch=(x, residual, a, b))
     nbytes = es * (M * Cin + M * Cout * (2 if residual is not None else 1) + Cout * Cin) + 4 * Cout
     meta = (f"gn_conv1x1<{'bf16' if es == 2 else 'f32'},{_tile_name(tile)}>[M={M},K={Cin},N={Cout}]", 2 * M * Cout * Cin, nbytes)
-    if stats is not None:
+    if fold is not None:
+        _dispatch("mmd_gn_conv1x1_stats_fold", *base, tile, *_stats_args(stats, M, Cout), ctypes.pointer(fold), meta=meta)
+    elif stats is not None:
         _dispatch("mmd_gn_conv1x1_stats", *base, tile, *_stats_args(stats, M, Cout), meta=meta)
     else:
         _dispatch("mmd_gn_conv1x1", *base, tile, meta=meta)
```

New measurement: 345.2 pair-steps/s (median of 2 runs). 0.985x the previous value.
